# PJLab-ADG/nr3d_lib

Hardware: AMD Instinct MI355X
Metric: Mpoints/s LoTD fwd+bwd (16-lvl hash) + Mrays/s march+composite, 1 & 8 GPU (higher is better)
Workload: dtype f32; 1 GPU; configs[1]: 16-level Hash LoTD (gen_ngp_cfg: T=2^19, F=2, 6 Dense + 10 Hash), 2^20 points/GPU, fwd(+dy/dx) + dL/dx + dL/dparam, fp32; points_per_gpu=1048576, n_params=12131648, parallelism=single GPU

## Files before the change

include/nr3d_hip.h:

```cpp
#ifndef NR3D_HIP_H
#define NR3D_HIP_H
#include <stdint.h>

#ifdef __cplusplus
extern "C" {
#endif

enum { NR3D_F32 = 0, NR3D_F16 = 1, NR3D_F64 = 2, NR3D_I32 = 3, NR3D_I64 = 4, NR3D_U8 = 5, NR3D_I16 = 6, NR3D_I8 = 7 };

#define NR3D_ABI_VERSION 16

const char *nr3d_last_error(void);
int nr3d_abi_version(void);

enum {
	NR3D_PROF_LOTD_FWD = 0,
	NR3D_PROF_LOTD_FWD_LDS = 1,
	NR3D_PROF_LOTD_CONTRACT_DX = 2,
	NR3D_PROF_LOTD_BIN = 3,
	NR3D_PROF_LOTD_ACCUM = 4,
	NR3D_PROF_MARCH = 5,
	NR3D_PROF_COMPOSITE_FWD = 6,
	NR3D_PROF_COMPOSITE_BWD = 7,
	NR3D_PROF_LOTD_DIRECT = 8,
	NR3D_PROF_COUNT = 9
};
void nr3d_prof_enable(uint32_t mask);
int nr3d_prof_read(int id, double *total_ms, uint32_t *n_intervals, int reset);

enum {
	NR3D_OPT_LOTD_PAIR = 0,
	NR3D_OPT_PAIR_QUAD = 1,
	NR3D_OPT_PAIR_SECOND = 2,
	NR3D_OPT_PAIR_DIRECT = 3,
	NR3D_OPT_PAIR_FIXED = 4,
	NR3D_OPT_FWD_PAIRLANE = 5,
	NR3D_OPT_FWD_SPLIT = 6,
	NR3D_OPT_FWD_LDS_STAGE = 7,
	NR3D_OPT_HVP_LEVELS = 8,
	NR3D_OPT_HVP_PAIRLANE = 9,
	NR3D_OPT_HVP_SPLIT = 10,
	NR3D_OPT_VM_SPLIT = 11,
	NR3D_OPT_CP_DIRECT = 12,
	NR3D_OPT_MARCH_GROUP = 13,
	NR3D_OPT_PACK_SCAN = 14,
	NR3D_OPT_SORT_WAVE = 15,
	NR3D_OPT_VM_DIRECT = 16,
	NR3D_OPT_DIRECT_FIXED = 17,
	NR3D_OPT_VM_SORTED = 18,
	NR3D_OPT_MLP_X3 = 19,
	NR3D_OPT_PAIR_FOLD = 20,
	NR3D_OPT_COUNT = 21
};
int nr3d_set_option(int id, int64_t value);
int64_t nr3d_get_option(int id);

#define NR3D_LOTD_MAX_LEVELS 32
#define NR3D_LOTD_MAX_DIMS 4
#define NR3D_LOTD_MAX_PSEUDO 256

enum {
	NR3D_LOD_Dense = 0, NR3D_LOD_VectorMatrix = 1, NR3D_LOD_VecZMatXoY = 2, NR3D_LOD_CP = 3,
	NR3D_LOD_CPfast = 4, NR3D_LOD_NPlaneMul = 5, NR3D_LOD_NPlaneSum = 6, NR3D_LOD_Hash = 7
};

typedef struct nr3d_lotd_level {
	uint32_t res[NR3D_LOTD_MAX_DIMS];
	uint32_t n_feats;
	uint32_t type;
	uint32_t size;
	uint32_t offset;
} nr3d_lotd_level_t;

typedef struct nr3d_lotd_meta {
	nr3d_lotd_level_t levels[NR3D_LOTD_MAX_LEVELS];
	uint16_t map_levels[NR3D_LOTD_MAX_PSEUDO];
	uint16_t map_cnt[NR3D_LOTD_MAX_PSEUDO];
	uint32_t n_levels;
	uint32_t n_pseudo_levels;
	uint32_t n_feat_per_pseudo_lvl;
	uint32_t n_dims_to_encode;
	uint32_t n_encoded_dims;
	uint32_t n_params;
	uint32_t interpolation_type;
	uint32_t c_hash_only;
	uint16_t map_col[NR3D_LOTD_MAX_PSEUDO];
} nr3d_lotd_meta_t;

int nr3d_lotd_meta_create(int32_t n_input_dim, uint32_t n_levels, const int32_t *res_multidim,
                          const int32_t *n_feats, const int32_t *types, uint32_t hashmap_size,
                          int use_smooth_step, nr3d_lotd_meta_t *out);

int nr3d_lotd_meta_regroup(const nr3d_lotd_meta_t *meta, uint32_t width, uint32_t max_width, nr3d_lotd_meta_t *out);


int nr3d_lotd_fwd(const nr3d_lotd_meta_t *meta, const void *meta_dev, uint32_t n_points,
                  int x_dtype, int param_dtype, const void *x, const void *params,
                  const int64_t *batch_inds, const int64_t *batch_offsets, uint32_t batch_data_size,
                  int32_t max_level, void *y, int64_t y_sn, int64_t y_se,
                  void *dy_dx, int64_t dydx_sn, int64_t dydx_se, void *stream);

int nr3d_lotd_bwd_dx(const nr3d_lotd_meta_t *meta, uint32_t n_points, int x_dtype, int param_dtype,
                     const void *dL_dy, int64_t dldy_sn, int64_t dldy_se,
                     const void *dy_dx, int64_t dydx_sn, int64_t dydx_se, void *dL_dx,
                     void *dL_dy_T ,
                     int32_t max_level, void *fold ,
                     void *stream);

uint64_t nr3d_lotd_dparam_workspace_bytes(const nr3d_lotd_meta_t *meta, uint32_t n_points, uint32_t n_batches);
void nr3d_lotd_set_dparam_chunk_log2(int log2_points);
int nr3d_lotd_bwd_dparam(const nr3d_lotd_meta_t *meta, const void *meta_dev, uint32_t n_points,
                         int x_dtype, int param_dtype, const void *dL_dy, int64_t dldy_sn, int64_t dldy_se,
                         const void *x, const void *params, const int64_t *batch_inds,
                         const int64_t *batch_offsets, uint32_t batch_data_size, uint32_t n_batches, int32_t max_level,
                         void *dL_dparam, void *workspace, uint64_t workspace_bytes, void *stream);
int nr3d_lotd_bwd_dparam_levels(const nr3d_lotd_meta_t *meta, const void *meta_dev, uint32_t n_points,
                                int x_dtype, int param_dtype, const void *dL_dy, int64_t dldy_sn, int64_t dldy_se,
                                const void *x, const void *params, const int64_t *batch_inds,
                                const int64_t *batch_offsets, uint32_t batch_data_size, uint32_t n_batches,
                                int32_t min_level, int32_t max_level, void *dL_dparam, void *workspace,
                                uint64_t workspace_bytes, void *stream);

int nr3d_lotd_dLdy_feature_major(uint32_t n_points, uint32_t n_encoded_dims, int grad_dtype, const void *dL_dy,
                                 int64_t g_sn, int64_t g_se, float *out, void *stream);

int nr3d_lotd_half_params_ok(const nr3d_lotd_meta_t *meta, int batched);
int nr3d_lotd_pair_path_ok(const nr3d_lotd_meta_t *meta);
int nr3d_lotd_pair_direct_levels(const nr3d_lotd_meta_t *meta, uint32_t n_points);
uint64_t nr3d_lotd_fwd_lds_levels(const nr3d_lotd_meta_t *meta, uint32_t n_points);
int nr3d_lotd_bwd_dparam_typed(const nr3d_lotd_meta_t *meta, const void *meta_dev, uint32_t n_points, int grad_dtype,
                               const void *dL_dy, int64_t g_sn, int64_t g_se, const void *x, int32_t max_level,
                               int out_dtype, int assign, void *dL_dparam, void *workspace, uint64_t workspace_bytes,
                               void *fold, void *stream);
uint64_t nr3d_lotd_pair_fold_bytes(const nr3d_lotd_meta_t *meta, uint32_t n_points, int32_t max_level);

int nr3d_lotd_bwd_bwd_ddLdy(const nr3d_lotd_meta_t *meta, uint32_t n_points, int x_dtype, int param_dtype,
                            const void *dL_ddLdx, const void *dy_dx, int64_t dydx_sn, int64_t dydx_se,
                            void *dL_ddLdy, int64_t out_sn, int64_t out_se, void *stream);
int nr3d_lotd_bwd_bwd_dparam(const nr3d_lotd_meta_t *meta, const void *meta_dev, uint32_t n_points,
                             int x_dtype, int param_dtype, const void *dL_ddLdx,
                             const void *dL_dy, int64_t dldy_sn, int64_t dldy_se, const void *x,
                             const void *params, const int64_t *batch_inds, const int64_t *batch_offsets,
                             uint32_t batch_data_size, uint32_t n_batches, int32_t max_level, void *dL_dparam,
                             void *workspace, uint64_t workspace_bytes, void *stream);
uint64_t nr3d_lotd_bwd_bwd_dx_workspace_bytes(const nr3d_lotd_meta_t *meta, uint32_t n_points);
int nr3d_lotd_bwd_bwd_dx(const nr3d_lotd_meta_t *meta, const void *meta_dev, uint32_t n_points,
                         int x_dtype, int param_dtype, const void *dL_ddLdx,
                         const void *dL_dy, int64_t dldy_sn, int64_t dldy_se, const void *x,
                         const void *params, const int64_t *batch_inds, const int64_t *batch_offsets,
                         uint32_t batch_data_size, int32_t max_level, void *dL_dx, void *workspace,
                         uint64_t workspace_bytes, void *stream);

int nr3d_lotd_grid_index(const nr3d_lotd_meta_t *meta, const void *meta_dev, uint32_t n_points, int x_dtype,
                         const void *x, const int64_t *batch_inds, const int64_t *batch_offsets,
                         uint32_t batch_data_size, int32_t max_level, int64_t *grid_inds, void *stream);

typedef struct nr3d_forest_meta {
	const uint8_t *octree;
	const int32_t *exsum;
	const int16_t *block_ks;
	float world_block_size[3];
	float world_origin[3];
	int32_t resolution[3];
	uint32_t n_trees;
	uint32_t level;
	uint32_t level_poffset;
	int32_t continuity_enabled;
} nr3d_forest_meta_t;

int nr3d_forest_identify(const nr3d_forest_meta_t *forest, uint64_t n, const int16_t *ks, int32_t *block_inds,
                         void *stream);

int nr3d_lotd_forest_fwd(const nr3d_lotd_meta_t *meta, const void *meta_dev, const nr3d_forest_meta_t *forest,
                         uint32_t n_points, const float *x, const void *params, int param_dtype ,
                         const int64_t *block_inds,
                         const int64_t *block_offsets, uint32_t batch_data_size, int32_t max_level, float *y,
                         int64_t y_sn, int64_t y_se, float *dy_dx, int64_t d_sn, int64_t d_se, void *stream);

uint64_t nr3d_lotd_forest_dparam_workspace_bytes(const nr3d_lotd_meta_t *meta, uint32_t n_points, uint32_t n_trees);
int nr3d_lotd_forest_bwd_dparam(const nr3d_lotd_meta_t *meta, const void *meta_dev, const nr3d_forest_meta_t *forest,
                                uint32_t n_points, const float *dL_ddLdx, const float *dL_dy, const float *x,
                                const void *params, int param_dtype, const int64_t *block_inds, const int64_t *block_offsets,
                                uint32_t batch_data_size, int32_t max_level, float *dL_dparam, void *workspace,
                                uint64_t workspace_bytes, void *stream);

int nr3d_lotd_forest_bwd_bwd_dx(const nr3d_lotd_meta_t *meta, const void *meta_dev, const nr3d_forest_meta_t *forest,
// ... 288 lines not shown
```

nr3d_lib_amd/_abi.py:

```python
ABI_VERSION = 16
SIGNATURES = {
    'nr3d_abi_version': ('int', []),
    'nr3d_alpha_to_vw_backward': ('int', ['uint32_t', 'uint64_t', 'ptr', 'ptr', 'ptr', 'ptr', 'float', 'float', 'ptr', 'ptr']),
    'nr3d_alpha_to_vw_forward': ('int', ['uint32_t', 'uint64_t', 'ptr', 'ptr', 'float', 'float', 'ptr', 'ptr', 'ptr', 'ptr']),
    'nr3d_arange_num_steps': ('int', ['uint32_t', 'int', 'ptr', 'ptr', 'ptr', 'double', 'ptr', 'ptr']),
    'nr3d_forest_identify': ('int', ['ptr', 'uint64_t', 'ptr', 'ptr', 'ptr']),
    'nr3d_forest_ray_marching_count': ('int', ['ptr', 'uint32_t', 'ptr', 'ptr', 'ptr', 'ptr', 'ptr', 'ptr', 'ptr', 'ptr', 'ptr', 'ptr', 'float', 'float', 'float', 'uint32_t', 'ptr', 'ptr', 'ptr', 'ptr']),
    'nr3d_forest_ray_marching_emit': ('int', ['ptr', 'uint32_t', 'ptr', 'ptr', 'ptr', 'ptr', 'ptr', 'ptr', 'ptr', 'ptr', 'ptr', 'ptr', 'float', 'float', 'float', 'ptr', 'ptr', 'ptr', 'ptr', 'ptr', 'ptr', 'ptr']),
    'nr3d_freq_encode_bwd': ('int', ['uint64_t', 'uint32_t', 'uint32_t', 'uint32_t', 'ptr', 'ptr', 'int64_t', 'ptr', 'ptr']),
    'nr3d_freq_encode_bwd_bwd': ('int', ['uint64_t', 'uint32_t', 'uint32_t', 'uint32_t', 'ptr', 'ptr', 'ptr', 'int64_t', 'ptr', 'ptr', 'ptr']),
    'nr3d_freq_encode_fwd': ('int', ['uint64_t', 'uint32_t', 'uint32_t', 'uint32_t', 'ptr', 'ptr', 'int64_t', 'ptr']),
    'nr3d_get_option': ('int64_t', ['int']),
    'nr3d_interleave_linstep': ('int', ['uint32_t', 'int', 'ptr', 'ptr', 'ptr', 'double', 'double', 'ptr', 'ptr', 'ptr']),
    'nr3d_last_error': ('str', []),
    'nr3d_lotd_bwd_bwd_ddLdy': ('int', ['ptr', 'uint32_t', 'int', 'int', 'ptr', 'ptr', 'int64_t', 'int64_t', 'ptr', 'int64_t', 'int64_t', 'ptr']),
    'nr3d_lotd_bwd_bwd_dparam': ('int', ['ptr', 'ptr', 'uint32_t', 'int', 'int', 'ptr', 'ptr', 'int64_t', 'int64_t', 'ptr', 'ptr', 'ptr', 'ptr', 'uint32_t', 'uint32_t', 'int32_t', 'ptr', 'ptr', 'uint64_t', 'ptr']),
    'nr3d_lotd_bwd_bwd_dx': ('int', ['ptr', 'ptr', 'uint32_t', 'int', 'int', 'ptr', 'ptr', 'int64_t', 'int64_t', 'ptr', 'ptr', 'ptr', 'ptr', 'uint32_t', 'int32_t', 'ptr', 'ptr', 'uint64_t', 'ptr']),
    'nr3d_lotd_bwd_bwd_dx_workspace_bytes': ('uint64_t', ['ptr', 'uint32_t']),
    'nr3d_lotd_bwd_dparam': ('int', ['ptr', 'ptr', 'uint32_t', 'int', 'int', 'ptr', 'int64_t', 'int64_t', 'ptr', 'ptr', 'ptr', 'ptr', 'uint32_t', 'uint32_t', 'int32_t', 'ptr', 'ptr', 'uint64_t', 'ptr']),
    'nr3d_lotd_bwd_dparam_levels': ('int', ['ptr', 'ptr', 'uint32_t', 'int', 'int', 'ptr', 'int64_t', 'int64_t', 'ptr', 'ptr', 'ptr', 'ptr', 'uint32_t', 'uint32_t', 'int32_t', 'int32_t', 'ptr', 'ptr', 'uint64_t', 'ptr']),
    'nr3d_lotd_bwd_dparam_typed': ('int', ['ptr', 'ptr', 'uint32_t', 'int', 'ptr', 'int64_t', 'int64_t', 'ptr', 'int32_t', 'int', 'int', 'ptr', 'ptr', 'uint64_t', 'ptr', 'ptr']),
    'nr3d_lotd_bwd_dx': ('int', ['ptr', 'uint32_t', 'int', 'int', 'ptr', 'int64_t', 'int64_t', 'ptr', 'int64_t', 'int64_t', 'ptr', 'ptr', 'int32_t', 'ptr', 'ptr']),
    'nr3d_lotd_dLdy_feature_major': ('int', ['uint32_t', 'uint32_t', 'int', 'ptr', 'int64_t', 'int64_t', 'ptr', 'ptr']),
    'nr3d_lotd_dparam_workspace_bytes': ('uint64_t', ['ptr', 'uint32_t', 'uint32_t']),
    'nr3d_lotd_forest_bwd_bwd_dx': ('int', ['ptr', 'ptr', 'ptr', 'uint32_t', 'ptr', 'ptr', 'ptr', 'ptr', 'int', 'ptr', 'ptr', 'uint32_t', 'int32_t', 'ptr', 'ptr']),
    'nr3d_lotd_forest_bwd_dparam': ('int', ['ptr', 'ptr', 'ptr', 'uint32_t', 'ptr', 'ptr', 'ptr', 'ptr', 'int', 'ptr', 'ptr', 'uint32_t', 'int32_t', 'ptr', 'ptr', 'uint64_t', 'ptr']),
    'nr3d_lotd_forest_dparam_workspace_bytes': ('uint64_t', ['ptr', 'uint32_t', 'uint32_t']),
    'nr3d_lotd_forest_fwd': ('int', ['ptr', 'ptr', 'ptr', 'uint32_t', 'ptr', 'ptr', 'int', 'ptr', 'ptr', 'uint32_t', 'int32_t', 'ptr', 'int64_t', 'int64_t', 'ptr', 'int64_t', 'int64_t', 'ptr']),
    'nr3d_lotd_fwd': ('int', ['ptr', 'ptr', 'uint32_t', 'int', 'int', 'ptr', 'ptr', 'ptr', 'ptr', 'uint32_t', 'int32_t', 'ptr', 'int64_t', 'int64_t', 'ptr', 'int64_t', 'int64_t', 'ptr']),
    'nr3d_lotd_fwd_lds_levels': ('uint64_t', ['ptr', 'uint32_t']),
    'nr3d_lotd_grid_index': ('int', ['ptr', 'ptr', 'uint32_t', 'int', 'ptr', 'ptr', 'ptr', 'uint32_t', 'int32_t', 'ptr', 'ptr']),
    'nr3d_lotd_half_params_ok': ('int', ['ptr', 'int']),
    'nr3d_lotd_meta_create': ('int', ['int32_t', 'uint32_t', 'ptr', 'ptr', 'ptr', 'uint32_t', 'int', 'ptr']),
    'nr3d_lotd_meta_regroup': ('int', ['ptr', 'uint32_t', 'uint32_t', 'ptr']),
    'nr3d_lotd_pair_direct_levels': ('int', ['ptr', 'uint32_t']),
    'nr3d_lotd_pair_fold_bytes': ('uint64_t', ['ptr', 'uint32_t', 'int32_t']),
    'nr3d_lotd_pair_path_ok': ('int', ['ptr']),
    'nr3d_lotd_set_dparam_chunk_log2': ('void', ['int']),
    'nr3d_march_composite_bwd': ('int', ['uint32_t', 'ptr', 'ptr', 'ptr', 'ptr', 'ptr', 'float', 'float', 'int', 'ptr', 'ptr', 'ptr', 'ptr', 'ptr', 'ptr', 'ptr', 'ptr', 'ptr', 'ptr', 'uint64_t', 'ptr', 'ptr']),
    'nr3d_march_composite_fwd': ('int', ['uint32_t', 'ptr', 'ptr', 'ptr', 'ptr', 'ptr', 'ptr', 'ptr', 'int', 'float', 'float', 'float', 'uint32_t', 'ptr', 'ptr', 'ptr', 'ptr', 'ptr', 'ptr', 'uint64_t', 'uint64_t', 'ptr', 'ptr', 'ptr', 'ptr', 'ptr', 'ptr', 'ptr', 'ptr', 'uint64_t', 'ptr', 'float', 'float', 'int', 'ptr', 'ptr', 'ptr', 'ptr', 'ptr', 'ptr']),
    'nr3d_march_finish_samples': ('int', ['uint64_t', 'ptr', 'ptr', 'ptr', 'ptr', 'ptr', 'ptr', 'ptr', 'ptr', 'ptr']),
    'nr3d_mark_pack_boundaries': ('int', ['uint64_t', 'int', 'ptr', 'ptr', 'ptr']),
    'nr3d_merge_pack_union': ('int', ['uint32_t', 'ptr', 'ptr', 'uint32_t', 'ptr', 'ptr', 'ptr', 'ptr', 'ptr', 'ptr', 'ptr', 'ptr', 'ptr', 'ptr', 'ptr', 'ptr']),
    'nr3d_mlp_backward': ('int', ['ptr', 'uint64_t', 'ptr', 'int64_t', 'int64_t', 'ptr', 'int64_t', 'ptr', 'ptr', 'int64_t', 'int64_t', 'ptr', 'ptr', 'ptr']),
    'nr3d_mlp_backward_backward': ('int', ['ptr', 'uint64_t', 'ptr', 'int64_t', 'int64_t', 'ptr', 'int64_t', 'ptr', 'int64_t', 'int64_t', 'ptr', 'ptr', 'int64_t', 'ptr', 'ptr']),
    'nr3d_mlp_backward_backward_ok': ('int', ['ptr']),
    'nr3d_mlp_backward_packed_floats': ('uint64_t', ['ptr']),
    'nr3d_mlp_forward': ('int', ['ptr', 'uint64_t', 'ptr', 'int64_t', 'int64_t', 'ptr', 'ptr', 'int64_t', 'ptr']),
    'nr3d_mlp_half_backward': ('int', ['ptr', 'uint64_t', 'ptr', 'int64_t', 'int64_t', 'ptr', 'int64_t', 'ptr', 'ptr', 'int64_t', 'int64_t', 'ptr', 'ptr', 'ptr']),
    'nr3d_mlp_half_backward_packed_bytes': ('uint64_t', ['ptr']),
    'nr3d_mlp_half_forward': ('int', ['ptr', 'uint64_t', 'ptr', 'int64_t', 'int64_t', 'ptr', 'ptr', 'int64_t', 'ptr']),
    'nr3d_mlp_half_pack': ('int', ['ptr', 'ptr', 'ptr', 'ptr', 'int', 'ptr']),
    'nr3d_mlp_half_packed_bytes': ('uint64_t', ['ptr']),
    'nr3d_mlp_pack': ('int', ['ptr', 'ptr', 'ptr', 'ptr', 'int', 'ptr']),
    'nr3d_mlp_packed_floats': ('uint64_t', ['ptr']),
    'nr3d_occ_apply_max': ('int', ['uint64_t', 'float', 'ptr', 'ptr', 'ptr']),
    'nr3d_occ_scatter_max': ('int', ['uint64_t', 'ptr', 'ptr', 'ptr', 'uint64_t', 'ptr', 'ptr', 'uint32_t', 'ptr', 'ptr']),
    'nr3d_octree_mark_consecutive_segments': ('int', ['uint32_t', 'ptr', 'ptr', 'ptr', 'ptr', 'ptr', 'ptr']),
    'nr3d_order_gather_inputs': ('int', ['uint32_t', 'ptr', 'ptr', 'ptr', 'ptr', 'ptr', 'ptr', 'ptr', 'ptr']),
    'nr3d_order_move_rows': ('int', ['uint32_t', 'ptr', 'int', 'ptr', 'uint32_t', 'ptr', 'ptr', 'uint32_t', 'ptr', 'ptr']),
    'nr3d_pack_composite_bwd': ('int', ['uint32_t', 'ptr', 'ptr', 'ptr', 'ptr', 'ptr', 'ptr', 'float', 'float', 'int', 'ptr', 'ptr', 'ptr', 'ptr', 'ptr', 'ptr', 'ptr', 'ptr', 'ptr', 'ptr']),
    'nr3d_pack_composite_fwd': ('int', ['uint32_t', 'ptr', 'ptr', 'ptr', 'ptr', 'ptr', 'float', 'float', 'int', 'ptr', 'ptr', 'ptr', 'ptr', 'ptr']),
    'nr3d_pack_infos_from_n': ('int', ['uint32_t', 'ptr', 'ptr', 'ptr', 'ptr', 'ptr']),
    'nr3d_packed_binary': ('int', ['uint32_t', 'uint64_t', 'uint32_t', 'uint32_t', 'int', 'ptr', 'ptr', 'ptr', 'int', 'int', 'ptr', 'ptr']),
    'nr3d_packed_diff': ('int', ['uint32_t', 'uint64_t', 'uint32_t', 'int', 'ptr', 'ptr', 'ptr', 'ptr', 'int', 'int', 'ptr', 'ptr']),
    'nr3d_packed_invert_cdf': ('int', ['uint32_t', 'ptr', 'ptr', 'ptr', 'ptr', 'uint32_t', 'ptr', 'ptr', 'ptr']),
    'nr3d_packed_scan': ('int', ['uint32_t', 'uint64_t', 'uint32_t', 'int', 'ptr', 'ptr', 'int', 'int', 'int', 'int', 'ptr', 'ptr']),
    'nr3d_packed_searchsorted': ('int', ['uint32_t', 'int', 'ptr', 'ptr', 'ptr', 'uint32_t', 'ptr', 'ptr', 'ptr']),
    'nr3d_packed_sort': ('int', ['uint32_t', 'uint64_t', 'int', 'ptr', 'ptr', 'ptr', 'ptr']),
    'nr3d_packed_sum': ('int', ['uint32_t', 'uint64_t', 'uint32_t', 'int', 'ptr', 'ptr', 'ptr', 'ptr']),
    'nr3d_permuto_bwd': ('int', ['ptr', 'uint32_t', 'int', 'ptr', 'int64_t', 'int64_t', 'ptr', 'ptr', 'ptr', 'ptr', 'ptr', 'ptr', 'uint32_t', 'int32_t', 'uint32_t', 'ptr', 'ptr', 'ptr']),
    'nr3d_permuto_bwd_bwd_input': ('int', ['ptr', 'uint32_t', 'int', 'ptr', 'ptr', 'int64_t', 'int64_t', 'ptr', 'ptr', 'ptr', 'ptr', 'ptr', 'ptr', 'uint32_t', 'int32_t', 'ptr', 'int64_t', 'int64_t', 'ptr', 'ptr']),
    'nr3d_permuto_fwd': ('int', ['ptr', 'uint32_t', 'int', 'ptr', 'ptr', 'ptr', 'ptr', 'ptr', 'ptr', 'uint32_t', 'int32_t', 'ptr', 'int64_t', 'int64_t', 'ptr']),
    'nr3d_permuto_meta_create': ('int', ['int32_t', 'int32_t', 'uint32_t', 'ptr', 'ptr', 'ptr', 'ptr']),
    'nr3d_permuto_supported_n_input_dims': ('int', ['ptr']),
    'nr3d_prof_enable': ('void', ['uint32_t']),
    'nr3d_prof_read': ('int', ['int', 'ptr', 'ptr', 'int']),
    'nr3d_prune_compact_packs': ('int', ['uint32_t', 'ptr', 'ptr', 'ptr', 'ptr', 'ptr', 'ptr', 'ptr', 'ptr']),
    'nr3d_prune_compact_samples': ('int', ['uint32_t', 'ptr', 'ptr', 'ptr', 'ptr', 'ptr', 'ptr', 'ptr', 'ptr', 'ptr', 'ptr', 'ptr', 'ptr', 'ptr']),
    'nr3d_ray_marching_cache_bytes': ('uint64_t', ['uint32_t', 'uint32_t']),
    'nr3d_ray_marching_count': ('int', ['uint32_t', 'ptr', 'ptr', 'ptr', 'ptr', 'ptr', 'ptr', 'ptr', 'int', 'float', 'float', 'float', 'uint32_t', 'int', 'ptr', 'uint32_t', 'ptr', 'ptr', 'ptr', 'ptr', 'uint64_t', 'ptr']),
    'nr3d_ray_marching_count_finished': ('int', ['uint32_t', 'ptr', 'ptr', 'ptr', 'ptr', 'ptr', 'ptr', 'ptr', 'int', 'float', 'float', 'float', 'uint32_t', 'int', 'ptr', 'uint32_t', 'ptr', 'ptr', 'ptr', 'ptr', 'ptr', 'ptr', 'uint64_t', 'ptr']),
    'nr3d_ray_marching_emit': ('int', ['uint32_t', 'ptr', 'ptr', 'ptr', 'ptr', 'ptr', 'ptr', 'ptr', 'int', 'float', 'float', 'float', 'int', 'ptr', 'uint32_t', 'ptr', 'ptr', 'ptr', 'ptr', 'ptr', 'ptr', 'ptr', 'uint32_t', 'ptr']),
    'nr3d_ray_marching_emit_finished': ('int', ['uint32_t', 'ptr', 'ptr', 'int', 'ptr', 'uint32_t', 'ptr', 'ptr', 'uint32_t', 'ptr', 'ptr', 'ptr', 'ptr', 'ptr', 'ptr', 'ptr', 'ptr', 'ptr']),
    'nr3d_sample_step_count': ('int', ['uint32_t', 'ptr', 'ptr', 'uint32_t', 'float', 'float', 'float', 'ptr', 'ptr']),
    'nr3d_sample_step_emit': ('int', ['uint32_t', 'ptr', 'ptr', 'float', 'float', 'float', 'ptr', 'ptr', 'ptr', 'ptr']),
    'nr3d_sample_step_segments': ('int', ['uint32_t', 'ptr', 'ptr', 'ptr', 'ptr', 'ptr', 'uint32_t', 'float', 'float', 'float', 'int', 'ptr', 'ptr', 'ptr', 'ptr', 'ptr', 'ptr', 'ptr']),
    'nr3d_scan_tmp_bytes': ('uint64_t', ['uint64_t']),
    'nr3d_set_option': ('int', ['int', 'int64_t']),
    'nr3d_sh_encode_bwd': ('int', ['uint64_t', 'uint32_t', 'uint32_t', 'int', 'ptr', 'int64_t', 'ptr', 'ptr', 'ptr', 'int', 'ptr']),
# ... 24 lines not shown
```

nr3d_lib_amd/_hip.py:

```python
import ctypes as C
import os
import subprocess
import threading

import torch

from nr3d_lib_amd import _abi

_PKG = os.path.dirname(os.path.abspath(__file__))
LIB_PATH = os.path.join(_PKG, "libnr3d_hip.so")
ABI_VERSION = _abi.ABI_VERSION
CSRC = os.path.join(_PKG, "csrc")

F32, F16, F64, I32, I64, U8, I16, I8 = range(8)
DTYPE_CODE = {
    torch.float32: F32, torch.float16: F16, torch.float64: F64, torch.int32: I32, torch.int64: I64,
    torch.uint8: U8, torch.bool: U8, torch.int16: I16, torch.int8: I8,
}

_lib = None
_lock = threading.Lock()


def build(verbose=False, jobs=None):
# ... 53 lines not shown
    if missing:
        raise RuntimeError(f"nr3d_lib_amd: {LIB_PATH} does not export {missing} (stale build? `make -C nr3d_lib_amd/csrc`)")


POISON = os.environ.get("NR3D_POISON_EMPTY", "0") == "1"


def _poison(t):
    if t.numel() == 0:
        return t
    if t.dtype.is_floating_point:
        t.fill_(float("nan"))
    elif t.dtype == torch.bool:
        t.fill_(True)
    else:
        t.fill_(-0x54545455 if t.dtype in (torch.int32, torch.int64) else 0x2B)
    return t


def empty(*args, **kwargs):
    t = torch.empty(*args, **kwargs)
    return _poison(t) if POISON else t


def empty_like(x, **kwargs):
    t = torch.empty_like(x, **kwargs)
    return _poison(t) if POISON else t


def check(rc):
    if rc != 0:
        raise RuntimeError(lib().nr3d_last_error().decode())


PROF_IDS = dict(lotd_fwd=0, lotd_fwd_lds=1, lotd_contract_dx=2, lotd_bin=3, lotd_accum=4, march=5, composite_fwd=6,
                composite_bwd=7, lotd_direct=8)


def prof_enable(*names):
    mask = 0
    for n in names:
        mask |= 1 << PROF_IDS[n]
    lib().nr3d_prof_enable(mask)


def prof_read(name, reset=True):
    ms, n = C.c_double(0.0), C.c_uint32(0)
    check(lib().nr3d_prof_read(PROF_IDS[name], C.byref(ms), C.byref(n), 1 if reset else 0))
    return float(ms.value), int(n.value)


OPTION_IDS = dict(lotd_pair=0, pair_quad=1, pair_second=2, pair_direct=3, pair_fixed=4, fwd_pairlane=5, fwd_split=6,
                  fwd_lds_stage=7, hvp_levels=8, hvp_pairlane=9, hvp_split=10, vm_split=11, cp_direct=12, march_group=13,
                  pack_scan=14, sort_wave=15, vm_direct=16, direct_fixed=17, vm_sorted=18, mlp_x3=19, pair_fold=20)


def set_option(name, value):
    l = lib()
    check(l.nr3d_set_option(OPTION_IDS[name], -1 if value is None else int(value)))


def get_option(name):
    l = lib()
    return int(l.nr3d_get_option(OPTION_IDS[name]))


class options:

    def __init__(self, **kw):
        self.kw, self.old = kw, {}

    def __enter__(self):
        for k, v in self.kw.items():
            self.old[k] = get_option(k)
            set_option(k, v)
        return self

    def __exit__(self, *a):
        for k, v in self.old.items():
            set_option(k, v)
        return False


def ptr(t):
    if t is None:
        return None
    return t.data_ptr()


_raw_stream = getattr(torch._C, "_cuda_getCurrentRawStream", None)


def stream_of(t):
    if _raw_stream is not None:
        return _raw_stream(t.device.index if t.device.index is not None else torch.cuda.current_device())
    return torch.cuda.current_stream(t.device).cuda_stream


def sort_pairs_u32(keys, values=None, bits=32, n_dev=None):
    pair = isinstance(keys, (list, tuple))
    ks = list(keys) if pair else [keys]
    vs = list(values) if isinstance(values, (list, tuple)) else [values] * len(ks)
    assert len(ks) in (1, 2) and all(k.is_cuda and k.dtype == torch.int32 and k.is_contiguous() and k.shape == ks[0].shape for k in ks)
    assert all(v is None or (v.is_cuda and v.dtype == torch.int32 and v.is_contiguous() and v.shape == ks[0].shape) for v in vs)
    n, dev = ks[0].numel(), ks[0].device
    l = lib()
    tmp = torch.empty(int(l.nr3d_sort_pairs_u32_tmp_bytes(n, len(ks))) or 1, dtype=torch.uint8, device=dev)
# ... 155 lines not shown
```

nr3d_lib_amd/bindings/_forest.py:

```python
import ctypes as C

import torch

from .. import _hip as H

__all__ = ['ForestMeta', 'forest_identify']


class _CForest(C.Structure):
    _fields_ = [("octree", C.c_void_p), ("exsum", C.c_void_p), ("block_ks", C.c_void_p),
                ("world_block_size", C.c_float * 3), ("world_origin", C.c_float * 3), ("resolution", C.c_int32 * 3),
                ("n_trees", C.c_uint32), ("level", C.c_uint32), ("level_poffset", C.c_uint32),
                ("continuity_enabled", C.c_int32)]


class ForestMeta:

    def __init__(self):
        self.octree = None
        self.exsum = None
        self.block_ks = None
        self.world_block_size = [1.0, 1.0, 1.0]
        self.world_origin = [0.0, 0.0, 0.0]
        self.resolution = [1, 1, 1]
# ... 68 lines not shown
            need_input_grad=None):
    from . import _lotd
    m, fo, N, bds = _check("fwd", metas, input, params, batch_inds, batch_offsets, batch_data_size)
    max_level = m.n_levels if max_level is None else int(max_level)
    need_input_grad = bool(input.requires_grad) if need_input_grad is None else bool(need_input_grad)
    E, dev = m.n_encoded_dims, input.device
    if max_level <= -1:
        return (torch.zeros((N, E), dtype=params.dtype, device=dev), torch.zeros((N, E * 3), dtype=input.dtype, device=dev))
    x32, (p32, pcode) = _lotd._f32c(input.detach()), _lotd._ptab(params)
    with H.on_device(dev):
        y = H.empty((E, N), dtype=torch.float32, device=dev).t()
        dy_dx, dsn, dse = None, 0, 0
        if need_input_grad:
            if m.c_permute_dydx:
                dy_dx = H.empty((E, N, 3), dtype=torch.float32, device=dev).permute(1, 0, 2)
                dsn, dse = dy_dx.stride(0), dy_dx.stride(1)
            else:
                dy_dx, dsn, dse = H.empty((N, E * 3), dtype=torch.float32, device=dev), E * 3, 3
        c = fo._c()
        H.check(H.lib().nr3d_lotd_forest_fwd(
            C.byref(m._cmeta()), H.ptr(m._dev(dev)), C.byref(c), N, H.ptr(x32), H.ptr(p32), pcode, H.ptr(batch_inds),
            H.ptr(batch_offsets), bds, max_level, H.ptr(y), y.stride(0), y.stride(1), H.ptr(dy_dx), dsn, dse, H.stream_of(input)))
    return _lotd._cast(y, params.dtype), _lotd._cast(dy_dx, input.dtype)


def lod_bwd(metas, dL_dy, input, params, dy_dx=None, batch_inds=None, batch_offsets=None, batch_data_size=None,
            max_level=None, need_input_grad=None, need_param_grad=None):
    from . import _lotd
    m, fo, N, bds = _check("bwd", metas, input, params, batch_inds, batch_offsets, batch_data_size)
    E, dev = m.n_encoded_dims, input.device
    H.require_gpu(dL_dy, dy_dx)
    if tuple(dL_dy.shape) != (N, E):
        raise RuntimeError(f"bwd: Expected dL_dy of size [{N}, {E}], got {list(dL_dy.shape)}")
    if dL_dy.dtype != params.dtype:
        raise RuntimeError("bwd: Expected dL_dy and grid to have the same dtype")
    max_level = m.n_levels if max_level is None else int(max_level)
    need_input_grad = bool(input.requires_grad) if need_input_grad is None else bool(need_input_grad)
    need_param_grad = bool(params.requires_grad) if need_param_grad is None else bool(need_param_grad)
    dL_dx = dL_dparam = None
    with H.on_device(dev):
        if need_input_grad:
            if dy_dx is None:
                raise RuntimeError("LoTDEncoding::bwd: need `dy_dx` to comput `dL_dx`.")
            dL_dx = torch.zeros((N, 3), dtype=torch.float32, device=dev)
        if need_param_grad:
            dL_dparam = torch.zeros((params.shape[0],), dtype=torch.float32, device=dev)
        if max_level <= -1 or N == 0 or not (need_input_grad or need_param_grad):
            return _lotd._cast(dL_dx, input.dtype), _lotd._cast(dL_dparam, params.dtype)
        g32 = _lotd._f32c(dL_dy.detach()).contiguous()
        st = H.stream_of(input)
        if need_input_grad:
            j, jsn, jse = _lotd._jac_view(dy_dx.detach(), N, E, 3)
            H.check(H.lib().nr3d_lotd_bwd_dx(
                C.byref(m._cmeta()), N, H.F32, H.F32, H.ptr(g32), E, 1, H.ptr(j), jsn, jse, H.ptr(dL_dx), None, max_level, None,
                st))
        if need_param_grad:
            x32, (p32, pcode) = _lotd._f32c(input.detach()), _lotd._ptab(params)
            c = fo._c()
            ws, wsb = _workspace(m, fo, N, dev)
            H.check(H.lib().nr3d_lotd_forest_bwd_dparam(
                C.byref(m._cmeta()), H.ptr(m._dev(dev)), C.byref(c), N, None, H.ptr(g32), H.ptr(x32), H.ptr(p32), pcode,
                H.ptr(batch_inds), H.ptr(batch_offsets), bds, max_level, H.ptr(dL_dparam), H.ptr(ws), wsb, st))
    return _lotd._cast(dL_dx, input.dtype), _lotd._cast(dL_dparam, params.dtype)


def lod_bwd_bwd_input(metas, dL_ddLdx, dL_dy, input, params, dy_dx=None, batch_inds=None, batch_offsets=None,
                      batch_data_size=None, max_level=None, need_dLdinput_ddLdoutput=None, need_dLdinput_dparams=None,
                      need_dLdinput_dinput=None):
    from . import _lotd
    m, fo, N, bds = _check("bwd_bwd_input", metas, input, params, batch_inds, batch_offsets, batch_data_size)
    E, dev = m.n_encoded_dims, input.device
    H.require_gpu(dL_ddLdx, dL_dy, dy_dx)
    if input.dtype != torch.float32:
        raise RuntimeError("LoTDEncoding: Input type combination not supported. Supported types are: "
                           "<input,param> -> (half, half), (float, half), (float, float)")
    if tuple(dL_ddLdx.shape) != (N, 3) or not dL_ddLdx.is_contiguous() or dL_ddLdx.dtype != input.dtype:
        raise RuntimeError(f"bwd_bwd_input: Expected contiguous dL_ddLdx of size [{N}, 3] and the input's dtype")
    if tuple(dL_dy.shape) != (N, E) or dL_dy.dtype != params.dtype:
        raise RuntimeError(f"bwd_bwd_input: Expected dL_dy of size [{N}, {E}] and the params' dtype")
    max_level = m.n_levels if max_level is None else int(max_level)
    need_dLdy = bool(dL_dy.requires_grad) if need_dLdinput_ddLdoutput is None else bool(need_dLdinput_ddLdoutput)
    need_dx = bool(input.requires_grad) if need_dLdinput_dinput is None else bool(need_dLdinput_dinput)
    need_dp = bool(params.requires_grad) if need_dLdinput_dparams is None else bool(need_dLdinput_dparams)
    dL_ddLdy = dL_dparams = dL_dx = None
    with H.on_device(dev):
        if need_dLdy:
            if dy_dx is None:
                raise RuntimeError("LoTDEncoding::bwd_bwd_input: need `dy_dx` to compute `dL_d(dLdy)`.")
            dL_ddLdy = torch.zeros((N, E), dtype=torch.float32, device=dev)
        if need_dx:
            dL_dx = torch.zeros((N, 3), dtype=torch.float32, device=dev)
        if need_dp:
            dL_dparams = torch.zeros((params.shape[0],), dtype=torch.float32, device=dev)
        if max_level <= -1 or N == 0 or not (need_dLdy or need_dx or need_dp):
            return _lotd._cast(dL_ddLdy, dL_dy.dtype), _lotd._cast(dL_dparams, params.dtype), _lotd._cast(dL_dx, input.dtype)
        st = H.stream_of(input)
        v32, g32 = _lotd._f32c(dL_ddLdx.detach()), _lotd._f32c(dL_dy.detach()).contiguous()
        x32, (p32, pcode) = _lotd._f32c(input.detach()), _lotd._ptab(params)
        cm, md, c = C.byref(m._cmeta()), H.ptr(m._dev(dev)), fo._c()
        if need_dLdy:
            j, jsn, jse = _lotd._jac_view(dy_dx.detach(), N, E, 3)
            H.check(H.lib().nr3d_lotd_bwd_bwd_ddLdy(
                cm, N, H.F32, H.F32, H.ptr(v32), H.ptr(j), jsn, jse, H.ptr(dL_ddLdy), E, 1, st))
        if need_dx:
            H.check(H.lib().nr3d_lotd_forest_bwd_bwd_dx(
                cm, md, C.byref(c), N, H.ptr(v32), H.ptr(g32), H.ptr(x32), H.ptr(p32), pcode, H.ptr(batch_inds),
                H.ptr(batch_offsets), bds, max_level, H.ptr(dL_dx), st))
# ... 11 lines not shown
```

nr3d_lib_amd/bindings/_lotd.py:

```python
import ctypes as C
import enum

import torch

from .. import _hip as H

MAX_LEVELS, MAX_DIMS, MAX_PSEUDO = 32, 4, 256


class LoDType(enum.IntEnum):
    Dense = 0
    VectorMatrix = 1
    VecZMatXoY = 2
    CP = 3
    CPfast = 4
    NPlaneMul = 5
    NPlaneSum = 6
    Hash = 7


class InterpolationType(enum.IntEnum):
    Linear = 0
    Smoothstep = 1

# ... 297 lines not shown
    if dy_dx is not None and input.dtype != torch.float32:
        dy_dx = dy_dx.to(input.dtype)
    return y, dy_dx


def lod_bwd(lod_meta, dL_dy, input, params, dy_dx=None, batch_inds=None, batch_offsets=None, batch_data_size=None,
            max_level=None, need_input_grad=None, need_param_grad=None, level_buckets=None, on_bucket=None):
    if isinstance(lod_meta, tuple):
        from . import _forest
        return _forest.lod_bwd(lod_meta, dL_dy, input, params, dy_dx, batch_inds, batch_offsets, batch_data_size, max_level,
                               need_input_grad, need_param_grad)
    m = lod_meta
    N, bds = _check_common("bwd", m, input, params, batch_inds, batch_offsets, batch_data_size)
    E, D = m.n_encoded_dims, m.n_dims_to_encode
    H.require_gpu(dL_dy, dy_dx)
    if dL_dy.dim() != 2 or tuple(dL_dy.shape) != (N, E):
        raise RuntimeError(f"bwd: Expected dL_dy of size [{N}, {E}], got {list(dL_dy.shape)}")
    if dL_dy.dtype != params.dtype:
        raise RuntimeError("bwd: Expected dL_dy and grid to have the same dtype")
    if dy_dx is not None and dy_dx.dtype != input.dtype:
        raise RuntimeError("bwd: Expected x and dy_dx to have the same dtype")
    max_level = m.n_levels if max_level is None else int(max_level)
    need_input_grad = bool(input.requires_grad) if need_input_grad is None else bool(need_input_grad)
    need_param_grad = bool(params.requires_grad) if need_param_grad is None else bool(need_param_grad)
    dev = input.device
    dL_dx = dL_dparam = None
    with H.on_device(dev):
        if need_input_grad and dy_dx is None:
            raise RuntimeError("LoTDEncoding::bwd: need `dy_dx` to comput `dL_dx`.")
        batched = batch_inds is not None or batch_offsets is not None or bds != 0
        nothing = max_level <= -1 or not (need_input_grad or need_param_grad) or N == 0
        native = (_native_half(m, params, batched) and level_buckets is None and USE_BINNED_DPARAM and input.dtype == torch.float32
                  and dL_dy.is_contiguous() and E % 4 == 0 and dL_dy.data_ptr() % 8 == 0 and not nothing
                  and params.shape[0] == m.n_params)
        typed = (not nothing and not batched and level_buckets is None and USE_BINNED_DPARAM
                 and (native or params.dtype == torch.float32) and params.shape[0] == m.n_params
                 and bool(H.lib().nr3d_lotd_pair_path_ok(C.byref(m._cmeta()))))
        if need_input_grad:
            dL_dx = (torch.zeros if nothing else H.empty)((N, D), dtype=torch.float32, device=dev)
        if need_param_grad:
            dL_dparam = (H.empty if typed else torch.zeros)((params.shape[0],), dtype=torch.float16 if native else torch.float32,
                                                                device=dev)
        if nothing:
            if need_param_grad and level_buckets is not None and on_bucket is not None:
                for k, (lo, hi) in enumerate(level_buckets):
                    on_bucket(k, dL_dparam[m.level_offsets[int(lo)]:m.level_offsets[min(int(hi), m.n_levels - 1) + 1]])
            return (_cast(dL_dx, input.dtype), _cast(dL_dparam, params.dtype))
        g32 = dL_dy.detach() if native else _f32c(dL_dy.detach())
        gcode = H.F16 if native else H.F32
        gsn, gse = _strides2(g32)
        st = H.stream_of(input)
        tag = ("dx" if need_input_grad else "") + ("dp" if need_param_grad else "")
        with _Prof(m, f"LoTD{D}-bwd-{tag}", N):
            gT = fold = None
            if need_input_grad and N > 0:
                j, jsn, jse = _jac_view(dy_dx.detach(), N, E, D)
                if (need_param_grad and not batched and USE_BINNED_DPARAM and gse == 1 and gsn == E
                        and g32.data_ptr() % 16 == 0):
                    gT = H.empty((E, N), dtype=torch.float32, device=dev)
                    if typed:
                        nfold = H.lib().nr3d_lotd_pair_fold_bytes(C.byref(m._cmeta()), N, max_level)
                        if nfold:
                            fold = H.empty(((nfold + 3) // 4,), dtype=torch.int32, device=dev)
                H.check(H.lib().nr3d_lotd_bwd_dx(
                    C.byref(m._cmeta()), N, H.F32, gcode, H.ptr(g32), gsn, gse, H.ptr(j), jsn, jse, H.ptr(dL_dx), H.ptr(gT),
                    max_level, H.ptr(fold), st))
            if need_param_grad and N > 0 and typed:
                ws, wsb = _dparam_workspace(m, N, dev, 1)
                if gT is not None:
                    g32, gsn, gse, gcode = gT, 1, N, H.F32
                H.check(H.lib().nr3d_lotd_bwd_dparam_typed(
                    C.byref(m._cmeta()), H.ptr(m._dev(dev)), N, gcode, H.ptr(g32), gsn, gse, H.ptr(_f32c(input.detach())),
                    max_level, H.F16 if native else H.F32, 1, H.ptr(dL_dparam), H.ptr(ws), wsb, H.ptr(fold), st))
            elif need_param_grad and N > 0:
                x32, (p32, pcode) = _f32c(input.detach()), _ptab(params)
                nbat = _n_batches(m, p32, batch_offsets, batched)
                ws, wsb = _dparam_workspace(m, N, dev, nbat)
                if gT is not None:
                    g32, gsn, gse = gT, 1, N
                if level_buckets is None:
                    H.check(H.lib().nr3d_lotd_bwd_dparam(
                        C.byref(m._cmeta()), H.ptr(m._dev(dev)), N, H.F32, pcode, H.ptr(g32), gsn, gse, H.ptr(x32), H.ptr(p32),
                        H.ptr(batch_inds), H.ptr(batch_offsets), bds, nbat, max_level, H.ptr(dL_dparam), H.ptr(ws), wsb, st))
                else:
                    if batched:
                        raise RuntimeError("bwd: level_buckets need non-batched params")
                    if params.dtype != torch.float32:
                        raise RuntimeError("bwd: level_buckets need float params (the slices handed out are the result)")
                    seen = set()
                    for k, (lo, hi) in enumerate(level_buckets):
                        lo, hi = int(lo), min(int(hi), m.n_levels - 1)
                        if lo < 0 or lo > hi or seen & set(range(lo, hi + 1)):
                            raise RuntimeError(f"bwd: bad or overlapping level bucket {(lo, hi)}")
                        seen |= set(range(lo, hi + 1))
                        H.check(H.lib().nr3d_lotd_bwd_dparam_levels(
                            C.byref(m._cmeta()), H.ptr(m._dev(dev)), N, H.F32, H.F32, H.ptr(g32), gsn, gse, H.ptr(x32), H.ptr(p32),
                            None, None, 0, nbat, lo, min(hi, max_level), H.ptr(dL_dparam), H.ptr(ws), wsb, st))
                        if on_bucket is not None:
                            on_bucket(k, dL_dparam[m.level_offsets[lo]:m.level_offsets[hi + 1]])
    return _cast(dL_dx, input.dtype), _cast(dL_dparam, params.dtype)


def _cast(t, dtype):
    if t is None or t.dtype == dtype:
        return t
    return t.to(dtype)


def lod_bwd_bwd_input(lod_meta, dL_ddLdx, dL_dy, input, params, dy_dx=None, batch_inds=None, batch_offsets=None,
                      batch_data_size=None, max_level=None, need_dLdinput_ddLdoutput=None,
                      need_dLdinput_dparams=None, need_dLdinput_dinput=None):
    if isinstance(lod_meta, tuple):
        from . import _forest
        return _forest.lod_bwd_bwd_input(lod_meta, dL_ddLdx, dL_dy, input, params, dy_dx, batch_inds, batch_offsets,
                                         batch_data_size, max_level, need_dLdinput_ddLdoutput, need_dLdinput_dparams,
                                         need_dLdinput_dinput)
    m = lod_meta
    N, bds = _check_common("bwd_bwd_input", m, input, params, batch_inds, batch_offsets, batch_data_size)
    E, D = m.n_encoded_dims, m.n_dims_to_encode
    H.require_gpu(dL_ddLdx, dL_dy, dy_dx)
    if input.dtype != torch.float32:
        raise RuntimeError("LoTDEncoding: Input type combination not supported. Supported types are: "
                           "<input,param> -> (half, half), (float, half), (float, float)")
    if tuple(dL_ddLdx.shape) != (N, D) or not dL_ddLdx.is_contiguous() or dL_ddLdx.dtype != input.dtype:
        raise RuntimeError(f"bwd_bwd_input: Expected contiguous dL_ddLdx of size [{N}, {D}] and the input's dtype")
    if tuple(dL_dy.shape) != (N, E) or dL_dy.dtype != params.dtype:
# ... 78 lines not shown
```

nr3d_lib_amd/csrc/host_api.hip:

```cpp
#include "common.h"
#include <string.h>
#include <limits>
#include <chrono>
#include <mutex>
#include <vector>

namespace nr3d {

static thread_local char g_err[512] = {0};

char *err_buf() { return g_err; }

int fail(const char *fmt, ...) {
	va_list ap;
	va_start(ap, fmt);
	vsnprintf(g_err, sizeof(g_err), fmt, ap);
	va_end(ap);
	return 1;
}

namespace prof {
uint32_t g_mask = 0;
struct Pair { hipEvent_t a, b; };
static std::mutex g_mu;
static std::vector<Pair> g_done[NR3D_PROF_COUNT];
static std::vector<Pair> g_free;
static Pair g_open[NR3D_PROF_COUNT];
static bool g_is_open[NR3D_PROF_COUNT] = {};

void begin(int id, hipStream_t st) {
	std::lock_guard<std::mutex> lk(g_mu);
	if (id < 0 || id >= NR3D_PROF_COUNT || g_is_open[id]) return;
	Pair p;
	if (!g_free.empty()) { p = g_free.back(); g_free.pop_back(); }
	else if (hipEventCreate(&p.a) != hipSuccess || hipEventCreate(&p.b) != hipSuccess) return;
	if (hipEventRecord(p.a, st) != hipSuccess) return;
	g_open[id] = p; g_is_open[id] = true;
}
void end(int id, hipStream_t st) {
	std::lock_guard<std::mutex> lk(g_mu);
	if (id < 0 || id >= NR3D_PROF_COUNT || !g_is_open[id]) return;
	g_is_open[id] = false;
	if (hipEventRecord(g_open[id].b, st) == hipSuccess) g_done[id].push_back(g_open[id]);
}
}

namespace opt {
static const int64_t kDefault[NR3D_OPT_COUNT] = {
	 1,  1,  1,  1,  1,  1,
	 1,  1,  1,  1,  1,  1,
	 1,  0,  1,  1,  1,  1,
	 1,  1,  1,
};
std::atomic<int64_t> g_val[NR3D_OPT_COUNT];
static const bool g_val_init = [] {
	for (int i = 0; i < NR3D_OPT_COUNT; ++i) g_val[i].store(kDefault[i], std::memory_order_relaxed);
	return true;
}();
}

}

using namespace nr3d;

extern "C" void nr3d_prof_enable(uint32_t mask) { prof::g_mask = mask; }

extern "C" int nr3d_prof_read(int id, double *total_ms, uint32_t *n_intervals, int reset) {
	NR3D_CHECK(id >= 0 && id < NR3D_PROF_COUNT && total_ms && n_intervals, "prof_read: bad argument");
	std::lock_guard<std::mutex> lk(prof::g_mu);
	double sum = 0.0;
	for (const prof::Pair &p : prof::g_done[id]) {
		NR3D_HIP_CHECK(hipEventSynchronize(p.b));
		float ms = 0.0f;
		NR3D_HIP_CHECK(hipEventElapsedTime(&ms, p.a, p.b));
		sum += ms;
	}
	*total_ms = sum;
	*n_intervals = (uint32_t)prof::g_done[id].size();
	if (reset) {
		for (const prof::Pair &p : prof::g_done[id]) prof::g_free.push_back(p);
		prof::g_done[id].clear();
	}
	return 0;
}

extern "C" int nr3d_set_option(int id, int64_t value) {
	NR3D_CHECK(id >= 0 && id < NR3D_OPT_COUNT, "nr3d_set_option: unknown option %d", id);
	opt::g_val[id].store(value < 0 ? opt::kDefault[id] : value, std::memory_order_relaxed);
	return 0;
}
extern "C" int64_t nr3d_get_option(int id) { return (id >= 0 && id < NR3D_OPT_COUNT) ? opt::get(id) : -1; }

extern "C" int nr3d_wait_host_words(const int64_t *words, int n, int64_t sentinel, uint32_t timeout_us) {
	if (!words || n <= 0) return 0;
	const auto t0 = std::chrono::steady_clock::now();
	for (uint32_t spin = 0;; ++spin) {
		bool all = true;
		for (int i = 0; i < n; ++i)
			if (__atomic_load_n(&words[i], __ATOMIC_ACQUIRE) == sentinel) { all = false; break; }
		if (all) return 0;
		__builtin_ia32_pause();
		if ((spin & 63u) == 63u &&
		    std::chrono::duration_cast<std::chrono::microseconds>(std::chrono::steady_clock::now() - t0).count() > (int64_t)timeout_us)
			return 1;
	}
// ... 129 lines not shown
```

nr3d_lib_amd/csrc/lotd.hip:

```cpp
#include "lotd_device.h"
#include <stdlib.h>
#include <vector>
#include <type_traits>
#include <algorithm>

namespace nr3d {
namespace lotd {

template <typename YT> __device__ __forceinline__ void store_nt(YT *p, float v);

template <int D, int G, bool DYDX, bool DH, int ONLY = -1, typename PT = float>
__global__ __launch_bounds__(kBlock) void k_fwd(Sched s, const nr3d_lotd_meta_t *__restrict__ md, uint32_t N,
                                                int32_t max_level, uint32_t smooth, const float *__restrict__ x,
                                                const PT *__restrict__ params, Batch ba, uint32_t vec_ok,
                                                PT *__restrict__ y, int64_t y_sn, int64_t y_se,
                                                float *__restrict__ dydx, int64_t d_sn, int64_t d_se) {
	uint32_t q, chunk;
	if (!decode_block(s, blockIdx.x, q, chunk)) return;
	const uint32_t i = chunk * kBlock + threadIdx.x;
	if (i >= N) return;
	const uint32_t level = meta_level_of(md, q);
	const uint32_t foff0 = meta_cnt_of(md, q) * G;
	const uint32_t out0 = meta_col_of(md, q);

// ... 955 lines not shown
			float *dst = reinterpret_cast<float *>(reinterpret_cast<char *>(partial) + ((size_t)q * N + g0) * 12u + pl * 12u);
			__builtin_nontemporal_store(ox[u], &dst[0]);
			__builtin_nontemporal_store(oy[u], &dst[1]);
			__builtin_nontemporal_store(oz[u], &dst[2]);
		}
	}
}

template <int D>
__global__ __launch_bounds__(kBlock) void k_sum_levels(uint32_t N, uint32_t n_pseudo, const float *__restrict__ partial,
                                                       float *__restrict__ dL_dx) {
	const uint32_t i = blockIdx.x * kBlock + threadIdx.x;
	if (i >= N) return;
	float acc[D];
#pragma unroll
	for (int d = 0; d < D; ++d) acc[d] = 0.0f;
	for (uint32_t q = 0; q < n_pseudo; ++q) {
		const float *src = partial + ((size_t)q * N + i) * D;
#pragma unroll
		for (int d = 0; d < D; ++d) acc[d] += __builtin_nontemporal_load(src + d);
	}
#pragma unroll
	for (int d = 0; d < D; ++d) dL_dx[(size_t)i * D + d] = acc[d];
}


template <int D>
__global__ __launch_bounds__(kBlock) void k_contract_dx(uint32_t N, uint32_t E, const float *__restrict__ dL_dy,
                                                        int64_t g_sn, int64_t g_se, const float *__restrict__ dydx,
                                                        int64_t d_sn, int64_t d_se, float *__restrict__ dL_dx) {
	const uint32_t i = blockIdx.x * kBlock + threadIdx.x;
	if (i >= N) return;
	float acc[D];
#pragma unroll
	for (int d = 0; d < D; ++d) acc[d] = 0.0f;
	const float *gy = dL_dy + (int64_t)i * g_sn;
	const float *jj = dydx + (int64_t)i * d_sn;
#pragma unroll 4
	for (uint32_t e = 0; e < E; ++e) {
		const float g = gy[(int64_t)e * g_se];
		const float *j = jj + (int64_t)e * d_se;
#pragma unroll
		for (int d = 0; d < D; ++d) acc[d] = __fmaf_rn(g, j[d], acc[d]);
	}
#pragma unroll
	for (int d = 0; d < D; ++d) dL_dx[(size_t)i * D + d] = acc[d];
}

template <int D, typename GT>
__global__ __launch_bounds__(kBlock) void k_contract_dx_rowmajor(uint32_t N, uint32_t E, const GT *__restrict__ dL_dy,
                                                                 const float *__restrict__ dydx, int64_t d_sn,
                                                                 int64_t d_se, float *__restrict__ dL_dx,
                                                                 float *__restrict__ dL_dy_T, uint32_t *__restrict__ fold,
                                                                 uint32_t gcols, uint32_t n_zero, uint32_t slot_off) {
	constexpr int TE = 32;
	__shared__ float tile[TE][kBlock + 1];
	__shared__ uint32_t gred[kBlock / 64];
	const uint32_t i0 = blockIdx.x * kBlock, i = i0 + threadIdx.x;
	const uint32_t n_here = min((uint32_t)kBlock, N - i0);
	uint32_t gbits = 0;
	auto gm = [&](uint32_t e, float v) { if (e < gcols) gbits = max(gbits, __float_as_uint(v) & 0x7FFFFFFFu); };
	if (fold && blockIdx.x == 0)
		for (uint32_t k = threadIdx.x; k < n_zero; k += kBlock) fold[k] = 0u;
	float acc[D];
#pragma unroll
	for (int d = 0; d < D; ++d) acc[d] = 0.0f;
	for (uint32_t e0 = 0; e0 < E; e0 += TE) {
		const uint32_t te = min((uint32_t)TE, E - e0);
		if (te == TE && (E & 3u) == 0u) {
#pragma unroll
			for (uint32_t v = threadIdx.x; v < kBlock * TE / 4; v += kBlock) {
				const uint32_t p = v >> 3, e4 = (v & 7u) * 4u;
				if (p < n_here) {
					float4 t;
					if constexpr (sizeof(GT) == 4) {
						t = *reinterpret_cast<const float4 *>(dL_dy + (size_t)(i0 + p) * E + e0 + e4);
					} else {
						const __half2 *h = reinterpret_cast<const __half2 *>(dL_dy + (size_t)(i0 + p) * E + e0 + e4);
						const float2 a = __half22float2(h[0]), b = __half22float2(h[1]);
						t = make_float4(a.x, a.y, b.x, b.y);
					}
					tile[e4][p] = t.x; tile[e4 + 1][p] = t.y; tile[e4 + 2][p] = t.z; tile[e4 + 3][p] = t.w;
					if (fold) { gm(e0 + e4, t.x); gm(e0 + e4 + 1, t.y); gm(e0 + e4 + 2, t.z); gm(e0 + e4 + 3, t.w); }
				}
			}
		} else {
			for (uint32_t v = threadIdx.x; v < kBlock * te; v += kBlock) {
				const uint32_t p = v / te, e = v - p * te;
				if (p < n_here) {
					tile[e][p] = to_f32<GT>(dL_dy[(size_t)(i0 + p) * E + e0 + e]);
					if (fold) gm(e0 + e, tile[e][p]);
				}
			}
		}
		__syncthreads();
		if (dL_dy_T && i < N) {
#pragma unroll 8
			for (uint32_t e = 0; e < te; ++e) __builtin_nontemporal_store(tile[e][threadIdx.x], &dL_dy_T[(size_t)(e0 + e) * N + i]);
		}
		if (i < N) {
			const float *jj = dydx + (int64_t)i * d_sn + (int64_t)e0 * d_se;
#pragma unroll 8
			for (uint32_t e = 0; e < te; ++e) {
				const float g = tile[e][threadIdx.x];
				const float *j = jj + (int64_t)e * d_se;
#pragma unroll
				for (int d = 0; d < D; ++d) acc[d] = __fmaf_rn(g, __builtin_nontemporal_load(j + d), acc[d]);
			}
		}
		__syncthreads();
	}
	if (i < N) {
#pragma unroll
		for (int d = 0; d < D; ++d) dL_dx[(size_t)i * D + d] = acc[d];
	}
	if (fold) {
#pragma unroll
		for (int off = 32; off >= 1; off >>= 1) gbits = max(gbits, (uint32_t)__shfl_xor((int)gbits, off, 64));
		if ((threadIdx.x & 63u) == 0) gred[threadIdx.x >> 6] = gbits;
		__syncthreads();
		if (threadIdx.x == 0) {
#pragma unroll
			for (int k = 1; k < kBlock / 64; ++k) gbits = max(gbits, gred[k]);
			fold[slot_off + blockIdx.x] = gbits;
		}
	}
}

template <int D>
__global__ __launch_bounds__(kBlock) void k_contract_ddLdy(uint32_t N, uint32_t E, const float *__restrict__ v,
                                                           const float *__restrict__ dydx, int64_t d_sn, int64_t d_se,
                                                           float *__restrict__ out, int64_t o_sn, int64_t o_se) {
	const uint32_t i = blockIdx.x * kBlock + threadIdx.x;
	const uint32_t e = blockIdx.y;
	if (i >= N) return;
	const float *j = dydx + (int64_t)i * d_sn + (int64_t)e * d_se;
	float r = 0.0f;
#pragma unroll
	for (int d = 0; d < D; ++d) r = __fmaf_rn(v[(size_t)i * D + d], j[d], r);
	out[(int64_t)i * o_sn + (int64_t)e * o_se] = r;
}

template <int D, int G>
__global__ __launch_bounds__(kBlock) void k_grid_index(Sched s, const nr3d_lotd_meta_t *__restrict__ md, uint32_t N,
                                                       uint32_t E, int32_t max_level, const float *__restrict__ x,
                                                       Batch ba, int64_t *__restrict__ out) {
	uint32_t q, chunk;
	if (!decode_block(s, blockIdx.x, q, chunk)) return;
	const uint32_t i = chunk * kBlock + threadIdx.x;
	if (i >= N) return;
	const uint32_t level = meta_level_of(md, q);
// ... 294 lines not shown
                       hipStream_t st) {
	uint32_t n_blocks;
	const Batch ba{batch_inds, batch_offsets, batch_data_size, meta->n_params};
	const uint32_t G = meta->n_feat_per_pseudo_lvl;
	const uint32_t elt = p_half ? 2u : 4u;
	const uint32_t vec_ok = (((uintptr_t)params % ((G >= 4 ? 4u : 2u) * elt)) == 0 && batch_offsets == nullptr) ? 1u : 0u;
	const bool dh = meta->c_hash_only != 0;
	prof::Scope ps(NR3D_PROF_LOTD_FWD, st);
	uint64_t grp[4] = {0, 0, 0, 0};
	const bool split = !dh && meta->n_pseudo_levels <= 64u && opt::on(NR3D_OPT_FWD_SPLIT);
	const uint64_t all = meta->n_pseudo_levels >= 64u ? ~0ull : ((1ull << meta->n_pseudo_levels) - 1ull);
	if (split) {
		for (uint32_t q = 0; q < meta->n_pseudo_levels; ++q) {
			const uint32_t t = meta->levels[meta->map_levels[q]].type;
			int k = 0;
			if (t == NR3D_LOD_Dense || t == NR3D_LOD_Hash) k = 1;
			else if (meta->n_dims_to_encode == 3 && t == NR3D_LOD_CP) k = 2;
			else if (meta->n_dims_to_encode == 3 && t == NR3D_LOD_VectorMatrix) k = 3;
			grp[k] |= 1ull << q;
		}
	} else {
		grp[dh ? 1 : 0] = all;
	}
	for (int k = 0; k < 4; ++k) {
		if (!grp[k]) continue;
		const uint64_t skip = (split || meta->n_pseudo_levels <= 64u) ? (all & ~grp[k]) : 0ull;
		const Sched s = make_sched(N, meta, n_blocks, skip);
		if (n_blocks == 0) continue;
		DISPATCH_DG(meta->n_dims_to_encode, G, {
			auto launch = [&](auto kern_f32, auto kern_f16) {
				if (p_half)
					hipLaunchKernelGGL(kern_f16, dim3(n_blocks), dim3(kBlock), 0, st, s, md, N, max_level,
					                   meta->interpolation_type, (const float *)x, (const __half *)params, ba, vec_ok,
					                   (__half *)y, y_sn, y_se, (float *)dy_dx, d_sn, d_se);
				else
					hipLaunchKernelGGL(kern_f32, dim3(n_blocks), dim3(kBlock), 0, st, s, md, N, max_level,
					                   meta->interpolation_type, (const float *)x, (const float *)params, ba, vec_ok,
					                   (float *)y, y_sn, y_se, (float *)dy_dx, d_sn, d_se);
			};
			if (k == 1) { if (dy_dx) NR3D_FWD2(D, true, true, -1); else NR3D_FWD2(D, false, true, -1); }
			else if (k == 0) { if (dy_dx) NR3D_FWD2(D, true, false, -1); else NR3D_FWD2(D, false, false, -1); }
			else if constexpr (D == 3) {
				if (k == 2) { if (dy_dx) NR3D_FWD2(3, true, false, NR3D_LOD_CP); else NR3D_FWD2(3, false, false, NR3D_LOD_CP); }
				else { if (dy_dx) NR3D_FWD2(3, true, false, NR3D_LOD_VectorMatrix); else NR3D_FWD2(3, false, false, NR3D_LOD_VectorMatrix); }
			}
		});
	}
	NR3D_LAUNCH_CHECK();
	return 0;
}

extern "C" int nr3d_lotd_bwd_dx(const nr3d_lotd_meta_t *meta, uint32_t N, int x_dtype, int param_dtype, const void *dL_dy,
                                int64_t g_sn, int64_t g_se, const void *dy_dx, int64_t d_sn, int64_t d_se, void *dL_dx,
                                void *dL_dy_T, int32_t max_level, void *fold_buf, void *stream) {
	NR3D_CHECK(meta != nullptr, "LoTD: meta is NULL");
	NR3D_CHECK(x_dtype == NR3D_F32 && (param_dtype == NR3D_F32 || param_dtype == NR3D_F16), "LoTD::bwd_dx: f32 x, f32 / f16 dL_dy");
	if (N == 0) return 0;
	NR3D_CHECK(dL_dy && dy_dx && dL_dx, "LoTDEncoding::bwd: need `dy_dx` to comput `dL_dx`.");
	const uint32_t E = meta->n_encoded_dims;
	const bool g_half = param_dtype == NR3D_F16;
	const bool row_major = (g_se == 1 && g_sn == (int64_t)E && ((uintptr_t)dL_dy % (g_half ? 8 : 16)) == 0);
	NR3D_CHECK(dL_dy_T == nullptr || row_major, "LoTD::bwd_dx: dL_dy_T needs a contiguous, 16-byte aligned [N, E] dL_dy");
	NR3D_CHECK(!g_half || (row_major && (E & 3u) == 0u), "LoTD::bwd_dx: half dL_dy must be a contiguous [N, E] tensor, E % 4 == 0");
	uint32_t gcols = 0, n_zero = 0, slot_off = 0;
	uint32_t *fold = (fold_buf && pair_fold_layout(meta, N, max_level, gcols, n_zero, slot_off) != 0) ? (uint32_t *)fold_buf : nullptr;
	NR3D_CHECK(!fold || row_major, "LoTD::bwd_dx: the hand-over buffer needs a contiguous, 16-byte aligned [N, E] dL_dy");
	prof::Scope ps(NR3D_PROF_LOTD_CONTRACT_DX, (hipStream_t)stream);
	DISPATCH_D(meta->n_dims_to_encode, {
		if (row_major && g_half)
			hipLaunchKernelGGL((k_contract_dx_rowmajor<D, __half>), dim3(div_up(N, kBlock)), dim3(kBlock), 0, (hipStream_t)stream, N, E,
			                   (const __half *)dL_dy, (const float *)dy_dx, d_sn, d_se, (float *)dL_dx, (float *)dL_dy_T, fold, gcols,
			                   n_zero, slot_off);
		else if (row_major)
			hipLaunchKernelGGL((k_contract_dx_rowmajor<D, float>), dim3(div_up(N, kBlock)), dim3(kBlock), 0, (hipStream_t)stream, N, E,
			                   (const float *)dL_dy, (const float *)dy_dx, d_sn, d_se, (float *)dL_dx, (float *)dL_dy_T, fold, gcols,
			                   n_zero, slot_off);
		else
			hipLaunchKernelGGL(k_contract_dx<D>, dim3(div_up(N, kBlock)), dim3(kBlock), 0, (hipStream_t)stream, N, E,
			                   (const float *)dL_dy, g_sn, g_se, (const float *)dy_dx, d_sn, d_se, (float *)dL_dx);
	});
	NR3D_LAUNCH_CHECK();
	return 0;
}

extern "C" uint64_t nr3d_lotd_pair_fold_bytes(const nr3d_lotd_meta_t *meta, uint32_t N, int32_t max_level) {
	uint32_t gcols, n_zero, slot_off;
	return meta ? pair_fold_layout(meta, N, max_level, gcols, n_zero, slot_off) : 0;
}

static int launch_bwd_dparam(const DparamPass &p) {
	const nr3d_lotd_meta_t *meta = p.meta;
	if (p.N == 0 || p.max_level <= -1 || p.min_level > p.max_level) return 0;
	NR3D_CHECK(p.dL_dy && p.x && p.params && p.dparam, "LoTD::bwd: NULL tensor pointer");
	const bool batched = p.batch.inds || p.batch.offsets || p.batch.data_size;
	if (p.workspace && (!batched || p.n_batches > 0)) {
		bool handled = false;
		DparamPass q = p;
		if (!batched) q.n_batches = 1u;
		NR3D_TRY(dparam_binned(q, handled));
		if (handled) return 0;
	}
	uint32_t n_blocks;
	const Sched s = make_sched(p.N, meta, n_blocks);
	const bool dh = meta->c_hash_only != 0;
	DISPATCH_DG(meta->n_dims_to_encode, meta->n_feat_per_pseudo_lvl, {
		auto launch = [&](auto kern, auto *tab) {
			hipLaunchKernelGGL(kern, dim3(n_blocks), dim3(kBlock), 0, p.st, s, p.meta_dev, p.N, p.min_level, p.max_level,
			                   meta->interpolation_type, p.dL_ddLdx, p.dL_dy, p.g_sn, p.g_se, p.x, tab, p.batch, p.dparam);
		};
		const float *pf = (const float *)p.params;
		if (dh || !p.p_half)
			with_bool(p.second, [&](auto S) { if (dh) launch(k_bwd_dparam<D, G, S(), true>, pf); else launch(k_bwd_dparam<D, G, S(), false>, pf); });
		else with_bool(p.second, [&](auto S) { launch(k_bwd_dparam<D, G, S(), false, __half>, (const __half *)p.params); });
	});
	NR3D_LAUNCH_CHECK();
	return 0;
}

extern "C" int nr3d_lotd_bwd_dparam(const nr3d_lotd_meta_t *meta, const void *meta_dev, uint32_t N, int x_dtype,
                                    int param_dtype, const void *dL_dy, int64_t g_sn, int64_t g_se, const void *x,
                                    const void *params, const int64_t *batch_inds, const int64_t *batch_offsets,
                                    uint32_t batch_data_size, uint32_t n_batches, int32_t max_level, void *dL_dparam,
                                    void *workspace, uint64_t workspace_bytes, void *stream) {
	if (int rc = check_common(meta, meta_dev, x_dtype, param_dtype, true)) return rc;
	DparamPass p = plain_pass(meta, meta_dev, N, dL_dy, g_sn, g_se, x, dL_dparam);
	p.params = params; p.p_half = param_dtype == NR3D_F16;
	p.batch = Batch{batch_inds, batch_offsets, batch_data_size, meta->n_params}; p.n_batches = n_batches;
	p.min_level = 0; p.max_level = max_level;
	p.workspace = workspace; p.workspace_bytes = workspace_bytes; p.st = (hipStream_t)stream;
	return launch_bwd_dparam(p);
}

extern "C" int nr3d_lotd_pair_path_ok(const nr3d_lotd_meta_t *meta) { return (meta && pair_applies(meta)) ? 1 : 0; }
extern "C" uint64_t nr3d_lotd_fwd_lds_levels(const nr3d_lotd_meta_t *meta, uint32_t n_points) {
	if (!meta || !pairlane_enabled() || !pairlane_meta_ok(meta)) return 0;
	return fwd_lds_levels(meta, n_points, 0x7fffffff);
}

extern "C" int nr3d_lotd_pair_direct_levels(const nr3d_lotd_meta_t *meta, uint32_t n_points) {
	return (meta && pair_applies(meta)) ? (int)pair_direct_levels(meta, n_points) : 0;
}

extern "C" int nr3d_lotd_bwd_dparam_typed(const nr3d_lotd_meta_t *meta, const void *meta_dev, uint32_t N, int grad_dtype,
                                          const void *dL_dy, int64_t g_sn, int64_t g_se, const void *x, int32_t max_level,
                                          int out_dtype, int assign, void *dL_dparam, void *workspace, uint64_t workspace_bytes,
                                          void *fold, void *stream) {
	if (int rc = check_common(meta, meta_dev, NR3D_F32, NR3D_F32)) return rc;
	NR3D_CHECK((grad_dtype == NR3D_F32 || grad_dtype == NR3D_F16) && (out_dtype == NR3D_F32 || out_dtype == NR3D_F16),
	           "LoTD::bwd_dparam_typed: f32 / f16 only");
	if (N == 0 || max_level <= -1) {
		if (assign && dL_dparam)
			NR3D_HIP_CHECK(hipMemsetAsync(dL_dparam, 0, (size_t)meta->n_params * (out_dtype == NR3D_F16 ? 2 : 4), (hipStream_t)stream));
		return 0;
	}
	NR3D_CHECK(dL_dy && x && dL_dparam && workspace, "LoTD::bwd: NULL tensor pointer");
	bool handled = false;
	DparamPass p = plain_pass(meta, meta_dev, N, dL_dy, g_sn, g_se, x, dL_dparam);
	p.g_half = grad_dtype == NR3D_F16; p.out_half = out_dtype == NR3D_F16; p.assign = assign != 0;
	p.max_level = max_level;
	p.workspace = workspace; p.workspace_bytes = workspace_bytes; p.st = (hipStream_t)stream;
	p.fold = (uint32_t *)fold;
	NR3D_TRY(dparam_binned(p, handled));
	NR3D_CHECK(handled, "LoTD::bwd_dparam_typed: the pair-record path does not apply to this meta / workspace");
	return 0;
}

extern "C" int nr3d_lotd_bwd_dparam_levels(const nr3d_lotd_meta_t *meta, const void *meta_dev, uint32_t N, int x_dtype,
                                           int param_dtype, const void *dL_dy, int64_t g_sn, int64_t g_se, const void *x,
                                           const void *params, const int64_t *batch_inds, const int64_t *batch_offsets,
                                           uint32_t batch_data_size, uint32_t n_batches, int32_t min_level,
                                           int32_t max_level, void *dL_dparam, void *workspace, uint64_t workspace_bytes,
                                           void *stream) {
	if (int rc = check_common(meta, meta_dev, x_dtype, param_dtype, true)) return rc;
	NR3D_CHECK(min_level >= 0, "LoTD::bwd: min_level must be >= 0");
	DparamPass p = plain_pass(meta, meta_dev, N, dL_dy, g_sn, g_se, x, dL_dparam);
	p.params = params; p.p_half = param_dtype == NR3D_F16;
	p.batch = Batch{batch_inds, batch_offsets, batch_data_size, meta->n_params}; p.n_batches = n_batches;
	p.min_level = min_level; p.max_level = max_level;
	p.workspace = workspace; p.workspace_bytes = workspace_bytes; p.st = (hipStream_t)stream;
	return launch_bwd_dparam(p);
}

extern "C" void nr3d_lotd_set_dparam_chunk_log2(int log2_points) { set_dparam_chunk_log2(log2_points); }

extern "C" uint64_t nr3d_lotd_dparam_workspace_bytes(const nr3d_lotd_meta_t *meta, uint32_t n_points, uint32_t n_batches) {
	return dparam_workspace_bytes(meta, n_points, n_batches);
}

extern "C" int nr3d_lotd_bwd_bwd_dparam(const nr3d_lotd_meta_t *meta, const void *meta_dev, uint32_t N, int x_dtype,
                                        int param_dtype, const void *dL_ddLdx, const void *dL_dy, int64_t g_sn,
                                        int64_t g_se, const void *x, const void *params, const int64_t *batch_inds,
                                        const int64_t *batch_offsets, uint32_t batch_data_size, uint32_t n_batches,
                                        int32_t max_level, void *dL_dparam, void *workspace, uint64_t workspace_bytes,
                                        void *stream) {
	if (int rc = check_common(meta, meta_dev, x_dtype, param_dtype, true)) return rc;
	NR3D_CHECK(N == 0 || dL_ddLdx != nullptr, "LoTD::bwd_bwd_input: dL_ddLdx is NULL");
	DparamPass p = plain_pass(meta, meta_dev, N, dL_dy, g_sn, g_se, x, dL_dparam);
	p.second = true; p.dL_ddLdx = (const float *)dL_ddLdx;
	p.params = params; p.p_half = param_dtype == NR3D_F16;
	p.batch = Batch{batch_inds, batch_offsets, batch_data_size, meta->n_params}; p.n_batches = n_batches;
	p.min_level = 0; p.max_level = max_level;
	p.workspace = workspace; p.workspace_bytes = workspace_bytes; p.st = (hipStream_t)stream;
	return launch_bwd_dparam(p);
}

extern "C" int nr3d_lotd_bwd_bwd_ddLdy(const nr3d_lotd_meta_t *meta, uint32_t N, int x_dtype, int param_dtype,
                                       const void *dL_ddLdx, const void *dy_dx, int64_t d_sn, int64_t d_se,
                                       void *dL_ddLdy, int64_t o_sn, int64_t o_se, void *stream) {
	NR3D_CHECK(meta != nullptr, "LoTD: meta is NULL");
	NR3D_CHECK(x_dtype == NR3D_F32 && param_dtype == NR3D_F32, "LoTD::bwd_bwd_ddLdy: f32 only");
	if (N == 0) return 0;
	NR3D_CHECK(dL_ddLdx && dy_dx && dL_ddLdy, "LoTDEncoding::bwd_bwd_input: need `dy_dx` to compute `dL_d(dLdy)`.");
	DISPATCH_D(meta->n_dims_to_encode, {
		hipLaunchKernelGGL(k_contract_ddLdy<D>, dim3(div_up(N, kBlock), meta->n_encoded_dims), dim3(kBlock), 0,
// ... 131 lines not shown
```

nr3d_lib_amd/csrc/lotd_bin.hip:

```cpp
#include "lotd_vm.h"
#include "lotd_sorted.h"
#include <stdlib.h>
#include <type_traits>

#ifndef NR3D_BIN_LDS_KB
#define NR3D_BIN_LDS_KB 72
#define NR3D_BIN_MAX_BP 512
#endif
namespace nr3d {
namespace lotd {

constexpr int kAccThreads = 1024;
constexpr int kLdsDoubles = 16384;
constexpr int kRedSlots = 4;
#ifndef NR3D_BALLOT_RANK_BUCKETS
#define NR3D_BALLOT_RANK_BUCKETS 4
#endif
constexpr uint32_t kBallotRankBuckets = NR3D_BALLOT_RANK_BUCKETS;
constexpr int kMaxPlanLevels = 64;
constexpr uint32_t kMaxBuckets = 8192;
constexpr int kBinLdsDyn = NR3D_BIN_LDS_KB * 1024 + (int)(kMaxBuckets + 1) * 4;

#define DISPATCH_DG_BIN(D_, G_, ...)                                                 \
	do {                                                                             \
// ... 1462 lines not shown
	}
	DISPATCH_DG_BIN(D, G, {
		if (meta->c_hash_only) {
			if constexpr (D <= 3) rc = launch_class<D, G, 8, true>(p, c, pl);
			else rc = launch_class<D, G, 16, true>(p, c, pl);
		} else if (cls == 8) rc = launch_class<D, G, 8, false>(p, c, pl);
		else if (cls == 16) {
			if constexpr (D >= 3) rc = launch_class<D, G, 16, false>(p, c, pl);
		} else if (cls == 24) {
			if constexpr (D == 3) rc = launch_class<D, G, 24, false>(p, c, pl);
		} else {
			if constexpr (D == 4) rc = launch_class<D, G, 32, false>(p, c, pl);
		}
	});
	return rc;
}

int dparam_binned(const DparamPass &pass, bool &handled) {
	handled = false;
	DparamPass p = pass;
	BinLayout lay;
	const uint32_t N = p.N, nc = chunk_points(N);
	const bool forest = p.forest != nullptr;
	nr3d_lotd_meta_t narrow;
	const bool narrowed = p.workspace && stage_a_meta(p.meta, forest, narrow);
	if (narrowed) p.meta = &narrow;
	const nr3d_lotd_meta_t *meta = p.meta;
	if (!p.workspace || !binnable(meta, forest) || !layout(meta, nc, p.n_batches, lay, forest)) return 0;
	if (p.workspace_bytes < lay.total + (narrowed ? kStageAMetaBytes : 0)) return 0;
	handled = true;
	char *ws = (char *)p.workspace;
	if (narrowed) {
		k_store_meta<<<1, 256, 0, p.st>>>(narrow, (uint32_t *)(ws + lay.total));
		NR3D_HIP_CHECK(hipGetLastError());
		p.meta_dev = (const nr3d_lotd_meta_t *)(ws + lay.total);
	}
	const uint32_t D = meta->n_dims_to_encode, E = meta->n_encoded_dims;
	DparamChunk c;
	c.rec = (uint32_t *)ws;
	c.offs = (uint32_t *)(ws + lay.rec_bytes);
	c.plan_buf = (uint32_t *)(ws + lay.rec_bytes + lay.offs_bytes);
	c.partial = (float *)(ws + lay.rec_bytes + lay.offs_bytes + lay.plan_bytes);
	c.gt = (float *)(ws + lay.rec_bytes + lay.offs_bytes + lay.plan_bytes + lay.part_bytes);
	c.dev = -1;
	const bool row_major = (p.g_se == 1 && p.g_sn == (int64_t)E && E > 1) || p.g_half;
	const bool plain = !forest && p.n_batches <= 1 && !p.batch.inds && !p.batch.offsets && !p.batch.data_size;
	const bool use_pair = plain && pair_applies(meta) && !(p.second && !pair_second_enabled());
	if ((p.g_half || p.out_half) && !use_pair)
		return ::nr3d::fail("LoTD::bwd: half gradients are served natively on the pair-record path only (nr3d_lotd_half_params_ok)");
	p.assign = pass.assign && use_pair && N <= nc && p.min_level <= 0 && p.max_level >= (int32_t)meta->n_levels - 1;
	if (pass.assign && !p.assign)
		NR3D_HIP_CHECK(hipMemsetAsync(p.dparam, 0, (size_t)(p.n_batches ? p.n_batches : 1u) * meta->n_params * (p.out_half ? 2 : 4), p.st));
	if (!(N <= nc && !p.second)) p.fold = nullptr;

	for (uint32_t p0 = 0; p0 < N; p0 += nc) {
		const uint32_t n = c.n = (N - p0) < nc ? (N - p0) : nc;
		c.xc = p.x + (size_t)p0 * D;
		c.vc = p.dL_ddLdx ? p.dL_ddLdx + (size_t)p0 * D : nullptr;
		c.g_rows = p.g_half ? reinterpret_cast<const float *>(reinterpret_cast<const __half *>(p.dL_dy) + (int64_t)p0 * p.g_sn)
		                    : p.dL_dy + (int64_t)p0 * p.g_sn;
		c.gc = c.g_rows;
		c.sn = p.g_sn; c.se = p.g_se;
		c.ba = p.batch;
		if (c.ba.inds) c.ba.inds += p0;
		c.ba.first_point = p0;
		bool gt_ready = !row_major;
		auto need_gt = [&]() {
			if (gt_ready) return;
			if (p.g_half) launch_transpose<__half>(n, E, reinterpret_cast<const __half *>(c.g_rows), p.g_sn, p.g_se, c.gt, p.st);
			else launch_transpose<float>(n, E, c.g_rows, p.g_sn, p.g_se, c.gt, p.st);
			c.gc = c.gt; c.sn = 1; c.se = (int64_t)n;
			gt_ready = true;
		};
		if (use_pair) {
			need_gt();
			NR3D_TRY(pair_chunk(p, c));
			continue;
		}
		uint64_t served = 0;
		if (plain) {
			CpPlan cp;
			uint32_t max_acc = 0;
			if ((served = cp_plan(meta, n, p.min_level, p.max_level, lay.part_bytes / 4, cp, max_acc))) {
				need_gt();
				NR3D_TRY(cp_direct_route(p, c, cp, max_acc));
			}
		}
		if (!p.g_half) {
			VsPlan vsp;
			const uint64_t smask = vm_sorted_plan(meta, n, p.n_batches, forest, p.min_level, p.max_level, served, vsp);
			if (smask) {
				VsScratch vss;
				vm_sorted_scratch(vsp, n, E, p.second, forest, vss);
				if (vss.total <= lay.rec_bytes + lay.offs_bytes) {
					NR3D_TRY(vm_sorted_run(p, c, vsp, vss));
					served |= smask;
				}
			}
		}
		if (plain) {
			VmPlan vp;
			const uint64_t vmask = vm_direct_plan(meta, n, p.min_level, p.max_level, lay.part_bytes / 4, vp, served);
			if (vmask) {
				need_gt();
				NR3D_TRY(vm_direct_route(p, c, vp));
				served |= vmask;
			}
		}
		for (uint32_t cls : kClasses) {
			BinPlan pl;
			uint64_t ow;
			make_plan(meta, n, p.n_batches, cls, PlanLevels{p.min_level, p.max_level, forest, served}, pl, ow);
			if (pl.n_pseudo == 0) continue;
			need_gt();
			NR3D_TRY(class_route(p, c, pl, cls));
		}
	}
	return 0;
}

}
}
```

nr3d_lib_amd/csrc/lotd_device.h:

```cpp
#pragma once
#include "common.h"
#include <type_traits>

namespace nr3d {
namespace lotd {

constexpr int kBlock = 256;
constexpr uint32_t kPrimes[7] = {1u, 2654435761u, 805459861u, 3674653429u, 2097192037u, 1434869437u, 2165219737u};

constexpr int kSchedSegs = 16;
struct Sched {
	uint32_t n_chunks, n_pseudo, mode, n_slots;
	uint64_t skip;
	uint32_t seg_cum[8][kSchedSegs + 1];
	uint32_t seg_begin[8][kSchedSegs];
	uint32_t seg_q[8][kSchedSegs];
};

__device__ __forceinline__ bool decode_block_raw(const Sched &s, uint32_t b, uint32_t &q, uint32_t &chunk);
__device__ __forceinline__ bool decode_block(const Sched &s, uint32_t b, uint32_t &q, uint32_t &chunk) {
	if (!decode_block_raw(s, b, q, chunk)) return false;
	return s.mode == 3 || q >= 64u || !((s.skip >> q) & 1ull);
}
__device__ __forceinline__ bool decode_block_raw(const Sched &s, uint32_t b, uint32_t &q, uint32_t &chunk) {
// ... 578 lines not shown
}

__device__ __forceinline__ bool resolve(const ForestDev &fo, const Batch &ba, const Lvl &L, const Block &b,
                                        const uint32_t (&p)[3], uint32_t (&pl)[3], uint32_t &offset) {
	uint32_t owner = 0xFFFFFFFFu;
	if (!resolve_block(fo, L, b.k, p, pl, owner)) return false;
	offset = (owner == 0xFFFFFFFFu) ? b.offset : (ba.offsets ? (uint32_t)ba.offsets[owner] : owner * ba.n_params);
	return true;
}

__device__ __forceinline__ void locate_forest(const float (&xp)[3], const Lvl &L, bool smooth, Cell<3> &c) {
#pragma unroll
	for (int d = 0; d < 3; ++d) {
		const float sc = (float)L.res[d];
		const float v = __fmaf_rn(xp[d], sc, 0.5f);
		const float fl = floorf(v);
		const float t = v - fl;
		c.sc[d] = sc;
		c.g[d] = (uint32_t)fl;
		if (!smooth) {
			c.w[d] = t; c.dw[d] = 1.0f; c.ddw[d] = 0.0f;
		} else {
			c.w[d] = t * t * __fmaf_rn(-2.0f, t, 3.0f);
			c.dw[d] = 6.0f * t * (1.0f - t);
			c.ddw[d] = __fmaf_rn(-12.0f, t, 6.0f);
		}
	}
}

uint64_t dparam_workspace_bytes(const nr3d_lotd_meta_t *m, uint32_t n_points, uint32_t n_batches, bool forest = false);
void set_dparam_chunk_log2(int lg);
struct DparamPass {
	bool second;
	const nr3d_lotd_meta_t *meta, *meta_dev;
	uint32_t N;
	const float *dL_ddLdx;
	const float *dL_dy;
	int64_t g_sn, g_se;
	bool g_half;
	const float *x;
	const void *params;
	bool p_half;
	Batch batch;
	uint32_t n_batches;
	int32_t min_level, max_level;
	float *dparam;
	bool out_half;
	bool assign;
	void *workspace;
	uint64_t workspace_bytes;
	hipStream_t st;
	const ForestDev *forest;
	uint32_t *fold;
};
struct DparamChunk {
	uint32_t n;
	const float *xc, *vc;
	const float *g_rows;
	const float *gc;
	int64_t sn, se;
	Batch ba;
	uint32_t *rec, *offs, *plan_buf;
	float *partial, *gt;
	int dev;
};

template <typename F> static inline void with_bool(bool b, F &&f) { if (b) f(std::true_type{}); else f(std::false_type{}); }
template <typename F> static inline void with_tables(const void *params, bool p_half, F &&f) {
	if (p_half) f((const __half *)params); else f((const float *)params);
}
template <typename P> using pointee_t = std::remove_const_t<std::remove_pointer_t<P>>;

static inline DparamPass plain_pass(const nr3d_lotd_meta_t *meta, const void *meta_dev, uint32_t N, const void *dL_dy, int64_t g_sn,
                                    int64_t g_se, const void *x, void *dparam) {
	DparamPass p;
	p.second = false; p.meta = meta; p.meta_dev = (const nr3d_lotd_meta_t *)meta_dev; p.N = N;
	p.dL_ddLdx = nullptr; p.dL_dy = (const float *)dL_dy; p.g_sn = g_sn; p.g_se = g_se; p.g_half = false;
	p.x = (const float *)x; p.params = nullptr; p.p_half = false;
	p.batch = Batch{nullptr, nullptr, 0u, meta->n_params}; p.n_batches = 1u;
	p.min_level = 0; p.max_level = 0x7fffffff;
	p.dparam = (float *)dparam; p.out_half = false; p.assign = false;
	p.workspace = nullptr; p.workspace_bytes = 0; p.st = nullptr;
	p.forest = nullptr; p.fold = nullptr;
	return p;
}

int dparam_binned(const DparamPass &pass, bool &handled);
bool dparam_one_pass(uint32_t n_points);

bool pair_applies(const nr3d_lotd_meta_t *m);
uint32_t pair_direct_levels(const nr3d_lotd_meta_t *m, uint32_t n_points);
void pair_layout(const nr3d_lotd_meta_t *m, uint32_t n_chunk, uint64_t &rec_bytes, uint64_t &offs_bytes, uint64_t &plan_bytes,
                 uint64_t &part_bytes);
int pair_chunk(const DparamPass &p, DparamChunk &c);
uint64_t pair_fold_layout(const nr3d_lotd_meta_t *m, uint32_t n, int32_t max_level, uint32_t &gcols, uint32_t &zero_words,
                          uint32_t &slot_off);

}
}
```

nr3d_lib_amd/csrc/lotd_pair.hip:

```cpp
#include "lotd_device.h"
#include <stdlib.h>


namespace nr3d {
namespace lotd {

constexpr uint32_t kPEpbMax = 8192;
constexpr int kPAccThreads = 1024;
constexpr int kPLdsMax = 2 * (int)kPEpbMax;
constexpr int kPMaxLv = 32;
constexpr uint32_t kPMaxNb = 511;
typedef uint32_t u32x4 __attribute__((ext_vector_type(4)));

struct PairPlan {
	uint32_t qmap[kPMaxLv];
	uint32_t nb[kPMaxLv];
	uint32_t epb[kPMaxLv];
	uint32_t shift[kPMaxLv];
	uint32_t bucket_base[kPMaxLv + 1];
	uint32_t offs_base[kPMaxLv];
	uint32_t n_blk, n_pseudo;
	uint32_t cap;
	uint32_t lg;
	uint32_t sum_log2;
};

constexpr uint32_t kDirectNb = 4, kDirectMaxLv = 8, kDirectMaxWg = 640;
struct DirectPlan {
	uint32_t n;
	uint32_t qmap[kDirectMaxLv], nb[kDirectMaxLv], epb[kDirectMaxLv], shift[kDirectMaxLv];
	uint32_t bucket_base[kDirectMaxLv + 1];
	uint32_t lg, sum_log2, R, pts_per_rep;
	uint32_t merge_min;
};


constexpr uint32_t kPairBp = 1024, kPairLg = 12, kPairUnroll = 4, kDirectRotate = 8, kPairUnits = 1536;
static bool pair_quad_enabled() { return opt::on(NR3D_OPT_PAIR_QUAD); }
static uint32_t pair_fixed() { return opt::on(NR3D_OPT_PAIR_FIXED) ? 1u : 0u; }

__device__ __forceinline__ float pair_wp2(float wp, float Cm, float Em, float &Cuse) {
	const float floor_c = fmaxf(1e-18f * fabsf(Em), 1e-30f);
	Cuse = !(fabsf(Cm) < floor_c) ? Cm : copysignf(floor_c, Cm);
	return __fmaf_rn(Em, __builtin_amdgcn_rcpf(Cuse), wp);
}
template <bool SECOND = false>
__device__ __forceinline__ void pair_records(const Lvl &L, uint32_t sh, uint32_t epb, uint32_t lg, const float (&xp)[3], float g0,
                                             float g1, bool smooth, uint32_t (&hdr)[4], uint32_t (&bkt)[4], float (&A)[4][2],
                                             float (&wpm)[SECOND ? 4 : 1], uint32_t (&cell)[3], uint32_t nb, bool &valid,
                                             const float *__restrict__ vin, uint32_t &qmask, float &wy, bool quad_on) {
	Cell<3> c;
	locate<3>(xp, L, smooth, c);
	valid = true;
	float a[3] = {0.0f, 0.0f, 0.0f};
	if constexpr (SECOND) {
#pragma unroll
		for (int d = 0; d < 3; ++d) a[d] = c.sc[d] * vin[d] * c.dw[d];
	}
	if constexpr (!SECOND) { qmask = 0; wy = c.w[1]; }
	if (L.type == NR3D_LOD_Dense) {
		const float wp = c.w[2];
#pragma unroll
		for (uint32_t m = 0; m < 4; ++m) {
			const uint32_t bx = m & 1u, by = m >> 1;
			const uint32_t row = (c.g[0] + bx) * L.res[1] + (c.g[1] + by);
			const uint32_t e0 = row * L.res[2] + c.g[2];
			const uint32_t b = row >> sh;
			const uint32_t i0 = e0 - b * epb;
			valid = valid && b < nb && c.g[2] + 1u < L.res[2];
			bkt[m] = b;
			hdr[m] = i0 | ((i0 + 1u) << 13);
			const float wx = bx ? c.w[0] : 1.0f - c.w[0], wy = by ? c.w[1] : 1.0f - c.w[1];
			const float wo = wx * wy;
			if constexpr (!SECOND) { A[m][0] = g0 * wo; A[m][1] = g1 * wo; wpm[0] = wp; }
			else {
				const float Cm = __fmaf_rn(bx ? a[0] : -a[0], wy, (by ? a[1] : -a[1]) * wx);
				float Cuse;
				wpm[m] = pair_wp2(wp, Cm, a[2] * wo, Cuse);
				A[m][0] = g0 * Cuse; A[m][1] = g1 * Cuse;
			}
		}
		if constexpr (!SECOND) {
#pragma unroll
			for (uint32_t bx = 0; bx < 2; ++bx)
				if (quad_on && bkt[bx] == bkt[bx + 2u] && (hdr[bx] & 8191u) + L.res[2] + 1u < 8192u) qmask |= 1u << bx;
		}
	} else {
		const float wp = c.w[0];
		const bool pow2 = (L.size & (L.size - 1u)) == 0u;
		const uint32_t emask = (1u << lg) - 1u;
#pragma unroll
		for (uint32_t m = 0; m < 4; ++m) {
			const uint32_t by = m & 1u, bz = m >> 1;
			const uint32_t K = ((c.g[1] + by) * kPrimes[1]) ^ ((c.g[2] + bz) * kPrimes[2]);
			const uint32_t h0 = c.g[0] ^ K, h1 = (c.g[0] + 1u) ^ K;
			const uint32_t e0 = pow2 ? (h0 & (L.size - 1u)) : (h0 % L.size);
			const uint32_t e1 = pow2 ? (h1 & (L.size - 1u)) : (h1 % L.size);
			bkt[m] = e0 >> lg;
			valid = valid && (e1 >> lg) == bkt[m] && bkt[m] < nb;
			hdr[m] = (e0 & emask) | ((e1 & emask) << 13);
			const float wy = by ? c.w[1] : 1.0f - c.w[1], wz = bz ? c.w[2] : 1.0f - c.w[2];
			const float wo = wy * wz;
			if constexpr (!SECOND) { A[m][0] = g0 * wo; A[m][1] = g1 * wo; wpm[0] = wp; }
			else {
				const float Cm = __fmaf_rn(by ? a[1] : -a[1], wz, (bz ? a[2] : -a[2]) * wy);
				float Cuse;
				wpm[m] = pair_wp2(wp, Cm, a[0] * wo, Cuse);
				A[m][0] = g0 * Cuse; A[m][1] = g1 * Cuse;
			}
		}
	}
#pragma unroll
	for (int d = 0; d < 3; ++d) cell[d] = c.g[d];
}

__device__ __forceinline__ void pair_buckets(const Lvl &L, uint32_t sh, uint32_t lg, const float (&xp)[3], bool smooth, uint32_t (&bkt)[4]) {
	Cell<3> c;
	locate<3>(xp, L, smooth, c);
	if (L.type == NR3D_LOD_Dense) {
#pragma unroll
		for (uint32_t m = 0; m < 4; ++m) bkt[m] = ((c.g[0] + (m & 1u)) * L.res[1] + (c.g[1] + (m >> 1))) >> sh;
	} else {
		const bool pow2 = (L.size & (L.size - 1u)) == 0u;
#pragma unroll
		for (uint32_t m = 0; m < 4; ++m) {
			const uint32_t h0 = c.g[0] ^ ((c.g[1] + (m & 1u)) * kPrimes[1]) ^ ((c.g[2] + (m >> 1)) * kPrimes[2]);
			bkt[m] = (pow2 ? (h0 & (L.size - 1u)) : (h0 % L.size)) >> lg;
		}
	}
}

template <int kPBP, bool SECOND = false>
__device__ __forceinline__ void pair_level(const PairPlan &plan, uint32_t ql, const Lvl &L, bool active, const float (&xp)[3],
                                           float g0, float g1, uint32_t smooth, u32x4 *__restrict__ stage,
                                           uint32_t *__restrict__ hist, uint32_t *__restrict__ zero_next, uint32_t *scan_lds,
                                           u32x4 *__restrict__ dst, uint32_t *__restrict__ ob, uint32_t ob_stride,
                                           const float *__restrict__ vin = nullptr, bool quad_on = false) {
	const uint32_t nb = plan.nb[ql];
	const uint32_t lane = threadIdx.x & 63u;
	uint32_t hdr[4], bkt[4], cell[3] = {0xFFFFFFFFu, 0xFFFFFFFFu, 0xFFFFFFFFu};
	constexpr int kW = SECOND ? 3 : 0;
	constexpr bool QUADS = !SECOND;
	uint32_t qmask = 0;
	float wy = 0.0f;
	float A[4][2], wp[SECOND ? 4 : 1];
#pragma unroll
	for (int m = 0; m < 4; ++m) { hdr[m] = 0; bkt[m] = 0; A[m][0] = 0.0f; A[m][1] = 0.0f; wp[m & kW] = 0.0f; }
	if (zero_next)
		for (uint32_t b = threadIdx.x; b <= kPMaxNb; b += kPBP) zero_next[b] = 0;
	if (active) {
		bool valid;
		pair_records<SECOND>(L, plan.shift[ql], plan.epb[ql], plan.lg, xp, g0, g1, smooth != 0, hdr, bkt, A, wp, cell, nb, valid, vin, qmask, wy,
		                     quad_on);
		active = valid;
	}

	bool emit = active, split = false;
	float Hh[4][2];
#pragma unroll
	for (int m = 0; m < 4; ++m) { Hh[m][0] = 0.0f; Hh[m][1] = 0.0f; }
	{
		auto prev = [](uint32_t v) { return (uint32_t)__builtin_amdgcn_update_dpp(0, (int)v, 0x138, 0xf, 0xf, false); };
		bool same = active && lane > 0;
#pragma unroll
		for (int d = 0; d < 3; ++d) same = same && (prev(cell[d]) == cell[d]);
		same = same && (prev((uint32_t)active) != 0u);
		const unsigned long long cont = __ballot(same);
		if (__popcll(cont) >= 16) {
			float lo[4][2], hi[4][2];
#pragma unroll
			for (int m = 0; m < 4; ++m)
#pragma unroll
				for (int f = 0; f < 2; ++f) { lo[m][f] = (1.0f - wp[m & kW]) * A[m][f]; hi[m][f] = wp[m & kW] * A[m][f]; }
#pragma unroll
			for (int off = 1; off < 64; off <<= 1) {
				const unsigned long long need = (1ull << off) - 1ull;
				const bool take = (lane + off < 64) && (((cont >> (lane + 1)) & need) == need);
#pragma unroll
				for (int m = 0; m < 4; ++m)
#pragma unroll
					for (int f = 0; f < 2; ++f) {
						const float tl = __shfl_down(lo[m][f], off, 64), th = __shfl_down(hi[m][f], off, 64);
						if (take) { lo[m][f] += tl; hi[m][f] += th; }
					}
			}
			const bool head_multi = active && !same && lane < 63 && ((cont >> (lane + 1)) & 1ull);
			if (same) emit = false;
			if (head_multi) {
// ... 7 lines not shown
	}

	uint32_t rank[4] = {0, 0, 0, 0};
	const uint32_t cnt = emit ? (split ? 2u : 1u) : 0u;
	auto emits = [&](int m) {
		if constexpr (QUADS) return emit && !(!split && m >= 2 && ((qmask >> (m - 2)) & 1u));
		else return emit;
	};
	if (nb <= 4) {
#pragma unroll
		for (int m = 0; m < 4; ++m) {
			const bool e_m = emits(m);
			const uint32_t bv = e_m ? bkt[m] : 0xFFFFFFFFu;
			unsigned long long todo = __ballot(e_m);
			while (todo) {
				const int leader = __ffsll((long long)todo) - 1;
				const uint32_t v = (uint32_t)__builtin_amdgcn_readlane((int)bv, leader);
				const bool mine = e_m && bv == v;
				const unsigned long long m1 = __ballot(mine), m2 = __ballot(mine && split);
				uint32_t first = 0;
				if ((int)lane == leader) first = atomicAdd(&hist[v], (uint32_t)(__popcll(m1) + __popcll(m2)));
				first = (uint32_t)__builtin_amdgcn_readlane((int)first, leader);
				const unsigned long long below = (1ull << lane) - 1ull;
				if (mine) rank[m] = first + (uint32_t)(__popcll(m1 & below) + __popcll(m2 & below));
				todo &= ~m1;
			}
		}
	} else {
#pragma unroll
		for (int m = 0; m < 4; ++m) {
			const bool e_m = emits(m);
			const uint32_t bv = e_m ? bkt[m] : 0xFFFFFFFFu;
			const unsigned long long em = __ballot(e_m);
			bool done = !e_m;
			if (em) {
				const int leader = __ffsll((long long)em) - 1;
				const uint32_t v = (uint32_t)__builtin_amdgcn_readlane((int)bv, leader);
				const bool mine = e_m && bv == v;
				const unsigned long long m1 = __ballot(mine);
				if (__popcll(m1) >= 8) {
					const unsigned long long m2 = __ballot(mine && split);
					uint32_t first = 0;
					if ((int)lane == leader) first = atomicAdd(&hist[v], (uint32_t)(__popcll(m1) + __popcll(m2)));
					first = (uint32_t)__builtin_amdgcn_readlane((int)first, leader);
					const unsigned long long below = (1ull << lane) - 1ull;
					if (mine) { rank[m] = first + (uint32_t)(__popcll(m1 & below) + __popcll(m2 & below)); done = true; }
				}
			}
			if (!done) rank[m] = atomicAdd(&hist[bv], cnt);
		}
	}
	__syncthreads();

	{
		const uint32_t b = threadIdx.x;
		const uint32_t v = (b < nb) ? hist[b] : 0u;
		uint32_t inc = v;
#pragma unroll
		for (int off = 1; off < 64; off <<= 1) {
			const uint32_t t = __shfl_up(inc, off, 64);
			if ((int)lane >= off) inc += t;
		}
		if (lane == 63) scan_lds[threadIdx.x >> 6] = inc;
		__syncthreads();
		uint32_t wave_off = 0;
#pragma unroll
		for (int k = 0; k < kPBP / 64; ++k) { const uint32_t t = scan_lds[k]; if (k < (int)(threadIdx.x >> 6)) wave_off += t; }
		if (b <= nb) hist[b] = wave_off + inc - v;
		__syncthreads();
	}

	if (emit) {
#pragma unroll
		for (int m = 0; m < 4; ++m) {
			if constexpr (QUADS) { if (!emits(m)) continue; }
			const uint32_t pos = hist[bkt[m]] + rank[m];
			if (QUADS && !split && m < 2 && ((qmask >> m) & 1u)) {
				const uint32_t wzq = (uint32_t)__float2uint_rn(wp[0] * 16777215.0f), wyq = (uint32_t)__float2uint_rn(wy * 16777215.0f);
				stage[pos] = u32x4{(hdr[m] & 8191u) | (((wyq >> 8) & 8191u) << 13) | (4u << 26) | ((wyq >> 21) << 29),
				                   wzq | ((wyq & 255u) << 24), __float_as_uint(A[m][0] + A[m + 2][0]), __float_as_uint(A[m][1] + A[m + 2][1])};
			} else if (!split) {
				stage[pos] = u32x4{hdr[m] | (3u << 26), __float_as_uint(wp[m & kW]), __float_as_uint(A[m][0]), __float_as_uint(A[m][1])};
			} else {
				stage[pos] = u32x4{(hdr[m] & 0x1FFFu) | (1u << 26), 0u, __float_as_uint(A[m][0]), __float_as_uint(A[m][1])};
				stage[pos + 1] = u32x4{(hdr[m] & 0x3FFE000u) | (2u << 26), 0u, __float_as_uint(Hh[m][0]), __float_as_uint(Hh[m][1])};
			}
		}
	}
	__syncthreads();

	const uint32_t total = hist[nb];
	for (uint32_t v = threadIdx.x; v < total; v += kPBP) __builtin_nontemporal_store(stage[v], dst + v);
	for (uint32_t b = threadIdx.x; b <= nb; b += kPBP) ob[(size_t)b * ob_stride] = hist[b];
	if (zero_next) __syncthreads();
}

template <int kPBP>
__device__ __forceinline__ void pair_gmax(uint32_t gbits, uint32_t *scan_lds, uint32_t *__restrict__ gmax) {
	const uint32_t lane = threadIdx.x & 63u;
#pragma unroll
	for (int off = 32; off >= 1; off >>= 1) gbits = max(gbits, (uint32_t)__shfl_xor((int)gbits, off, 64));
	__syncthreads();
	if (lane == 0) scan_lds[threadIdx.x >> 6] = gbits;
	__syncthreads();
	if (threadIdx.x == 0) {
		uint32_t m = 0;
#pragma unroll
		for (int k = 0; k < kPBP / 64; ++k) m = max(m, scan_lds[k]);
		if (m > __hip_atomic_load(gmax, __ATOMIC_RELAXED, __HIP_MEMORY_SCOPE_AGENT)) atomicMax(gmax, m);
	}
}

template <int kPBP, bool SECOND = false>
__global__ __launch_bounds__(kPBP, kPBP == 768 ? 6 : 8)  void k_pair_bin(PairPlan plan, const nr3d_lotd_meta_t *__restrict__ md, uint32_t n,
                                                   int32_t max_level, uint32_t smooth, const float *__restrict__ x,
                                                   const float *__restrict__ g, int64_t g_sn, int64_t g_se,
                                                   u32x4 *__restrict__ rec, uint32_t *__restrict__ offs_g,
                                                   uint32_t *__restrict__ gmax, DirectPlan dp, const float *__restrict__ vin_,
                                                   uint32_t quad_on) {
	constexpr uint32_t kPCap = (uint32_t)kPBP * 4u;
	extern __shared__ __attribute__((aligned(16))) uint32_t smem[];
	__shared__ uint32_t scan_lds[kPBP / 64];
	u32x4 *stage = reinterpret_cast<u32x4 *>(smem);
	uint32_t *hist = smem + (size_t)kPCap * 4;
	const uint32_t blk = blockIdx.x, ql = blockIdx.y;
	const uint32_t q = plan.qmap[ql], nb = plan.nb[ql];
	const uint32_t level = meta_level_of(md, q);
	const Lvl L = load_level(md, level);
	const uint32_t i = blk * kPBP + threadIdx.x;
	for (uint32_t b = threadIdx.x; b <= nb; b += kPBP) hist[b] = 0;
	__syncthreads();
	const bool active = (i < n) && ((int32_t)level <= max_level);
	float xp[3] = {0.0f, 0.0f, 0.0f}, vin[3] = {0.0f, 0.0f, 0.0f}, g0 = 0.0f, g1 = 0.0f;
	if (active) {
#pragma unroll
		for (int d = 0; d < 3; ++d) xp[d] = x[(size_t)i * 3 + d];
		g0 = g[(int64_t)i * g_sn + (int64_t)(q * 2) * g_se];
		g1 = g[(int64_t)i * g_sn + (int64_t)(q * 2 + 1) * g_se];
		if constexpr (SECOND) {
#pragma unroll
			for (int d = 0; d < 3; ++d) vin[d] = vin_[(size_t)i * 3 + d];
		}
	}
	pair_level<kPBP, SECOND>(plan, ql, L, active, xp, g0, g1, smooth, stage, hist, nullptr, scan_lds,
	                         rec + ((size_t)ql * plan.n_blk + blk) * (size_t)plan.cap, offs_g + plan.offs_base[ql] + blk, plan.n_blk, vin,
	                         quad_on != 0u);
	if (gmax) {
		uint32_t gbits;
		if constexpr (!SECOND) {
			gbits = max(__float_as_uint(g0) & 0x7FFFFFFFu, __float_as_uint(g1) & 0x7FFFFFFFu);
			if (ql == 0 && i < n)
				for (uint32_t e = 0; e < dp.n; ++e) {
					const uint32_t qd = dp.qmap[e];
					if ((int32_t)meta_level_of(md, qd) > max_level) continue;
					gbits = max(gbits, __float_as_uint(g[(int64_t)i * g_sn + (int64_t)(qd * 2) * g_se]) & 0x7FFFFFFFu);
					gbits = max(gbits, __float_as_uint(g[(int64_t)i * g_sn + (int64_t)(qd * 2 + 1) * g_se]) & 0x7FFFFFFFu);
				}
		} else {
			auto bound = [&](const Lvl &Lq, float ga, float gb) {
				const float m = __uint_as_float(max(__float_as_uint(ga) & 0x7FFFFFFFu, __float_as_uint(gb) & 0x7FFFFFFFu)) * 1.5f *
				                ((float)(Lq.res[0] - 2u) * fabsf(vin[0]) + (float)(Lq.res[1] - 2u) * fabsf(vin[1]) + (float)(Lq.res[2] - 2u) * fabsf(vin[2]));
				return __float_as_uint(m) & 0x7FFFFFFFu;
			};
			gbits = bound(L, g0, g1);
			if (ql == 0 && i < n) {
				if (!active) {
#pragma unroll
					for (int d = 0; d < 3; ++d) vin[d] = vin_[(size_t)i * 3 + d];
				}
				for (uint32_t e = 0; e < dp.n; ++e) {
					const uint32_t qd = dp.qmap[e];
					if ((int32_t)meta_level_of(md, qd) > max_level) continue;
					const Lvl Ld = load_level(md, meta_level_of(md, qd));
					gbits = max(gbits, bound(Ld, g[(int64_t)i * g_sn + (int64_t)(qd * 2) * g_se], g[(int64_t)i * g_sn + (int64_t)(qd * 2 + 1) * g_se]));
				}
			}
		}
		pair_gmax<kPBP>(gbits, scan_lds, gmax);
	}
}

__device__ __forceinline__ uint32_t gmax_slots(const uint32_t *__restrict__ slots, uint32_t n_slots, uint32_t *red) {
	uint32_t m = 0;
	for (uint32_t k = threadIdx.x; k < n_slots; k += 1024u) m = max(m, slots[k]);
#pragma unroll
	for (int off = 32; off >= 1; off >>= 1) m = max(m, (uint32_t)__shfl_xor((int)m, off, 64));
	__syncthreads();
	if ((threadIdx.x & 63u) == 0) red[threadIdx.x >> 6] = m;
	__syncthreads();
	m = 0;
#pragma unroll
	for (int k = 0; k < 16; ++k) m = max(m, red[k]);
	__syncthreads();
	return m;
}

__device__ __forceinline__ void pair_plan_block(const PairPlan &plan, const uint32_t *__restrict__ offs_g, uint32_t n_units,
                                                uint32_t *__restrict__ tot, uint32_t *__restrict__ rep,
                                                uint32_t *__restrict__ item_start, uint32_t *__restrict__ ticket, uint32_t bid,
                                                uint32_t nblk, const uint32_t *__restrict__ slots, uint32_t n_slots,
                                                uint32_t *__restrict__ gmax_out, bool empty_one) {
	__shared__ uint64_t red[16];
	__shared__ uint64_t carry_s;
	__shared__ uint32_t last_s;
	const uint32_t lane = threadIdx.x & 63, wave = threadIdx.x >> 6;
	const uint32_t NB = plan.bucket_base[plan.n_pseudo];
	{
		const uint32_t fb = bid * 16 + wave;
		if (fb < NB) {
			uint32_t q = 0;
			while (q + 1 < plan.n_pseudo && plan.bucket_base[q + 1] <= fb) ++q;
			const uint32_t *ob0 = offs_g + plan.offs_base[q] + (size_t)(fb - plan.bucket_base[q]) * plan.n_blk;
			const uint32_t *ob1 = ob0 + plan.n_blk;
			uint32_t sum = 0;
			for (uint32_t blk = lane; blk < plan.n_blk; blk += 64) sum += ob1[blk] - ob0[blk];
#pragma unroll
			for (int off = 32; off >= 1; off >>= 1) sum += __shfl_xor(sum, off, 64);
			if (lane == 0) __hip_atomic_store(tot + fb, sum, __ATOMIC_RELAXED, __HIP_MEMORY_SCOPE_AGENT);
		}
	}
	__syncthreads();
	if (threadIdx.x == 0) {
		__builtin_amdgcn_fence(__ATOMIC_RELEASE, "agent");
		asm volatile("s_waitcnt vmcnt(0)" ::: "memory");
		last_s = (atomicAdd(ticket, 1u) == nblk - 1u) ? 1u : 0u;
		__builtin_amdgcn_fence(__ATOMIC_ACQUIRE, "agent");
	}
	__syncthreads();
	if (!last_s) return;
	if (slots) {
		const uint32_t gb = gmax_slots(slots, n_slots, reinterpret_cast<uint32_t *>(red));
		if (threadIdx.x == 0) gmax_out[0] = gb;
	}
	auto ld_tot = [&](uint32_t fb) { return (uint64_t)__hip_atomic_load(tot + fb, __ATOMIC_RELAXED, __HIP_MEMORY_SCOPE_AGENT); };
	uint64_t part = 0;
	for (uint32_t fb = threadIdx.x; fb < NB; fb += 1024) part += ld_tot(fb);
#pragma unroll
	for (int off = 32; off >= 1; off >>= 1) part += __shfl_xor(part, off, 64);
	if (lane == 0) red[wave] = part;
	__syncthreads();
	uint64_t total = 0;
#pragma unroll
	for (int w = 0; w < 16; ++w) total += red[w];
	const uint64_t unit = total / n_units > 0 ? total / n_units : 1;
	if (threadIdx.x == 0) carry_s = 0;
	__syncthreads();
	for (uint32_t base = 0; base < NB; base += 1024) {
		const uint32_t fb = base + threadIdx.x;
		uint32_t r = 0;
		if (fb < NB) {
			const uint64_t t = ld_tot(fb);
			r = t == 0 ? (empty_one ? 1u : 0u) : (uint32_t)((t + unit / 2) / unit);
			if (t != 0 && r < 1) r = 1;
			if (r > plan.n_blk) r = plan.n_blk;
			rep[fb] = r;
		}
		uint64_t inc = r;
#pragma unroll
		for (int off = 1; off < 64; off <<= 1) { const uint64_t t2 = __shfl_up(inc, off, 64); if ((int)lane >= off) inc += t2; }
		__syncthreads();
		if (lane == 63) red[wave] = inc;
		__syncthreads();
		uint64_t woff = 0, tsum = 0;
#pragma unroll
		for (int w = 0; w < 16; ++w) { if (w < (int)wave) woff += red[w]; tsum += red[w]; }
		const uint64_t c = carry_s;
		if (fb < NB) item_start[fb] = (uint32_t)(c + woff + inc - r);
		__syncthreads();
// ... 66 lines not shown
	const uint32_t b = fb - dp.bucket_base[e], q = dp.qmap[e];
	const Lvl L = load_level(md, meta_level_of(md, q));
	const uint32_t foff0 = meta_cnt_of(md, q) * 2u, kPLds = 2u << dp.lg;
	if (t >= kPLds) return;
	float *p = pair_target(L, dp.epb[e], dp.lg, foff0, b, t, dparam, half_out);
	if (!p) return;
	const float sum = pair_replica_sum(dpart + (size_t)fb * dp.R * kPLds + t, dp.R, kPLds);
	pair_st(p, (assign ? 0.0f : pair_ld(p, half_out)) + sum, half_out);
}

template <int kUnroll, bool FIX>
__global__ __launch_bounds__(kPAccThreads, 8)  void k_pair_accum(PairPlan plan, const nr3d_lotd_meta_t *__restrict__ md,
                                                             const u32x4 *__restrict__ rec,
                                                             const uint32_t *__restrict__ offs_g,
                                                             const uint32_t *__restrict__ rep_g,
                                                             const uint32_t *__restrict__ item_start,
                                                             const uint32_t *__restrict__ gmax,
                                                             float *__restrict__ partial, float *__restrict__ dparam,
                                                             uint32_t out_half, uint32_t *__restrict__ bticket, uint32_t n_dred,
                                                             DirectPlan dp, const float *__restrict__ dpart) {
	extern __shared__ __attribute__((aligned(16))) unsigned long long acc_raw[];
	__shared__ uint32_t last_s;
	if (blockIdx.x < n_dred) {
		const uint32_t rows = (2u << dp.lg) / kPAccThreads;
		pair_direct_sum(dp, md, dpart, dparam, out_half, blockIdx.x / rows, (blockIdx.x % rows) * kPAccThreads + threadIdx.x);
		return;
	}
	const uint32_t item = blockIdx.x - n_dred;
	double *acc = reinterpret_cast<double *>(acc_raw);
	const uint32_t NB = plan.bucket_base[plan.n_pseudo];
	const cu32_t istart = (cu32_t)item_start, irep = (cu32_t)rep_g;
	if (item >= istart[NB]) return;
	uint32_t lo = 0, hi = NB;
	while (hi - lo > 1) { const uint32_t mid = (lo + hi) >> 1; if (istart[mid] <= item) lo = mid; else hi = mid; }
	const uint32_t fb = lo, R = irep[fb], r = item - istart[fb];
	uint32_t q = 0;
	while (q + 1 < plan.n_pseudo && plan.bucket_base[q + 1] <= fb) ++q;
	const uint32_t b = fb - plan.bucket_base[q];
	const uint32_t qg = plan.qmap[q];
	const Lvl L = load_level(md, meta_level_of(md, qg));
	const uint32_t foff0 = meta_cnt_of(md, qg) * 2u, epb = plan.epb[q];
	PairFix fx = {1.0, 1.0, false};
	if constexpr (FIX) fx = pair_fix(gmax, plan.sum_log2);
	const bool fix = FIX && fx.on;

	const uint32_t kPEpb = 1u << plan.lg, kPLds = 2u << plan.lg;
	for (uint32_t t = threadIdx.x; t < kPLds; t += kPAccThreads) acc_raw[t] = 0ull;
	__syncthreads();

	const uint32_t lane = threadIdx.x & 63, wave = threadIdx.x >> 6;
	constexpr uint32_t n_waves = kPAccThreads / 64;
	const uint32_t blk_lo = 0u, blk_hi = (plan.n_blk > r) ? (plan.n_blk - r + R - 1u) / R : 0u;
	const uint32_t *ob0 = offs_g + plan.offs_base[q] + (size_t)b * plan.n_blk;
	const uint32_t *ob1 = ob0 + plan.n_blk;
	const uint32_t kPCap = plan.cap;
	const u32x4 *rec_q = rec + (size_t)q * plan.n_blk * (size_t)kPCap;
	const uint32_t per_wave = (blk_hi - blk_lo + n_waves - 1) / n_waves;
	const uint32_t w_lo = min(blk_lo + wave * per_wave, blk_hi), w_hi = min(w_lo + per_wave, blk_hi);
	constexpr int kGroup = 8;
	for (uint32_t blk0 = w_lo; blk0 < w_hi; blk0 += 64) {
		const uint32_t mb = blk0 + lane;
		const uint32_t s_l = (mb < w_hi) ? ob0[r + R * mb] : 0u;
		const uint32_t e_l = (mb < w_hi) ? ob1[r + R * mb] : 0u;
		const uint32_t n_run = min(64u, w_hi - blk0);
		const u32x4 *rec_b = rec_q + (size_t)(r + R * blk0) * kPCap;
		for (uint32_t j0 = 0; j0 < n_run; j0 += kGroup) {
			uint32_t pre[kGroup + 1], rbase[kGroup];
			pre[0] = 0;
#pragma unroll
			for (int u = 0; u < kGroup; ++u) {
				const uint32_t j = min(j0 + (uint32_t)u, 63u);
				const uint32_t s_j = __builtin_amdgcn_readlane(s_l, j), e_j = __builtin_amdgcn_readlane(e_l, j);
				const uint32_t nrec = (j0 + (uint32_t)u < n_run) ? e_j - s_j : 0u;
				rbase[u] = s_j + j * R * kPCap - pre[u];
				pre[u + 1] = pre[u] + nrec;
			}
			const uint32_t total = pre[kGroup];
			for (uint32_t p0 = 0; p0 < total; p0 += 64u * kUnroll) {
				u32x4 rv[kUnroll];
#pragma unroll
				for (int v = 0; v < kUnroll; ++v) {
					const uint32_t pos = p0 + 64u * (uint32_t)v + lane;
					uint32_t at = rbase[0];
#pragma unroll
					for (int u = 1; u < kGroup; ++u) at = (pos >= pre[u]) ? rbase[u] : at;
					rv[v] = __builtin_nontemporal_load(rec_b + (size_t)(pos < total ? at + pos : rbase[0]));
				}
#pragma unroll
				for (int v = 0; v < kUnroll; ++v)
					if (p0 + 64u * (uint32_t)v + lane < total) {
						const uint32_t h = rv[v].x, fl = (h >> 26) & 7u;
						const uint32_t i0 = h & 8191u, i1 = (h >> 13) & 8191u;
						const float w = __uint_as_float(rv[v].y), a0 = __uint_as_float(rv[v].z), a1 = __uint_as_float(rv[v].w);
						if (fl == 4u) {
							const uint32_t wyq = (((h >> 13) & 8191u) << 8) | (rv[v].y >> 24) | ((h >> 29) << 21), wzq = rv[v].y & 0xFFFFFFu;
							const float wy = (float)wyq * (1.0f / 16777215.0f), wz = (float)wzq * (1.0f / 16777215.0f);
							const float q00 = (1.0f - wy) * (1.0f - wz), q01 = (1.0f - wy) * wz, q10 = wy * (1.0f - wz), q11 = wy * wz;
							const uint32_t i2 = i0 + L.res[2];
							if (fix) {
								atomicAdd(&acc_raw[i0], to_fix(q00 * a0, fx.scale)); atomicAdd(&acc_raw[kPEpb + i0], to_fix(q00 * a1, fx.scale));
								atomicAdd(&acc_raw[i0 + 1u], to_fix(q01 * a0, fx.scale)); atomicAdd(&acc_raw[kPEpb + i0 + 1u], to_fix(q01 * a1, fx.scale));
								atomicAdd(&acc_raw[i2], to_fix(q10 * a0, fx.scale)); atomicAdd(&acc_raw[kPEpb + i2], to_fix(q10 * a1, fx.scale));
								atomicAdd(&acc_raw[i2 + 1u], to_fix(q11 * a0, fx.scale)); atomicAdd(&acc_raw[kPEpb + i2 + 1u], to_fix(q11 * a1, fx.scale));
							} else {
								atomicAdd(&acc[i0], (double)(q00 * a0)); atomicAdd(&acc[kPEpb + i0], (double)(q00 * a1));
								atomicAdd(&acc[i0 + 1u], (double)(q01 * a0)); atomicAdd(&acc[kPEpb + i0 + 1u], (double)(q01 * a1));
								atomicAdd(&acc[i2], (double)(q10 * a0)); atomicAdd(&acc[kPEpb + i2], (double)(q10 * a1));
								atomicAdd(&acc[i2 + 1u], (double)(q11 * a0)); atomicAdd(&acc[kPEpb + i2 + 1u], (double)(q11 * a1));
							}
							continue;
						}
						const bool pair = fl == 3u;
						const float wl = pair ? 1.0f - w : 1.0f, wh = pair ? w : 1.0f;
						if (fix) {
							if (fl & 1u) { atomicAdd(&acc_raw[i0], to_fix(wl * a0, fx.scale)); atomicAdd(&acc_raw[kPEpb + i0], to_fix(wl * a1, fx.scale)); }
							if (fl & 2u) { atomicAdd(&acc_raw[i1], to_fix(wh * a0, fx.scale)); atomicAdd(&acc_raw[kPEpb + i1], to_fix(wh * a1, fx.scale)); }
// ... 40 lines not shown
		float *p[kFlush];
		float v[kFlush], old[kFlush];
#pragma unroll
		for (int k = 0; k < kFlush; ++k) {
			const uint32_t t = tb + (uint32_t)k * kPAccThreads;
			p[k] = (t < kPLds) ? pair_target(L, epb, plan.lg, foff0, b, t, dparam, (out_half & 1u) != 0) : nullptr;
			v[k] = p[k] ? value(t) : 0.0f;
		}
		const bool half_out = (out_half & 1u) != 0, assign = (out_half & 2u) != 0;
#pragma unroll
		for (int k = 0; k < kFlush; ++k) old[k] = (p[k] && !assign) ? pair_ld(p[k], half_out) : 0.0f;
#pragma unroll
		for (int k = 0; k < kFlush; ++k) if (p[k]) pair_st(p[k], old[k] + v[k], half_out);
	}
}

template <bool FIX, bool SECOND = false>
__global__ __launch_bounds__(kPAccThreads, 8) void k_pair_direct(DirectPlan dp, const nr3d_lotd_meta_t *__restrict__ md, uint32_t n,
                                                                 int32_t max_level, uint32_t smooth, const float *__restrict__ x,
                                                                 const float *__restrict__ g, int64_t g_sn, int64_t g_se,
                                                                 const uint32_t *__restrict__ gmax, float *__restrict__ partial,
                                                                 const float *__restrict__ vin_, uint32_t plan_rows, PairPlan plan,
                                                                 const uint32_t *__restrict__ offs_g, uint32_t n_units,
                                                                 uint32_t *__restrict__ tot, uint32_t *__restrict__ rep,
                                                                 uint32_t *__restrict__ item_start, uint32_t *__restrict__ ticket,
                                                                 const uint32_t *__restrict__ slots, uint32_t n_slots,
                                                                 uint32_t *__restrict__ gmax_out, uint32_t empty_one) {
	extern __shared__ __attribute__((aligned(16))) unsigned long long acc_raw[];
	__shared__ uint32_t queue[kPAccThreads / 64][128];
	if (blockIdx.y >= gridDim.y - plan_rows) {
		const uint32_t bid = (blockIdx.y - (gridDim.y - plan_rows)) * gridDim.x + blockIdx.x, nblk = (plan.bucket_base[plan.n_pseudo] + 15u) / 16u;
		if (bid < nblk) pair_plan_block(plan, offs_g, n_units, tot, rep, item_start, ticket, bid, nblk, slots, n_slots, gmax_out, empty_one != 0u);
		return;
	}
	double *acc = reinterpret_cast<double *>(acc_raw);
	const uint32_t r = blockIdx.x, fb = blockIdx.y;
	uint32_t e = 0;
	while (e + 1 < dp.n && dp.bucket_base[e + 1] <= fb) ++e;
	const uint32_t b = fb - dp.bucket_base[e], q = dp.qmap[e];
	const uint32_t level = meta_level_of(md, q);
	const Lvl L = load_level(md, level);
	const uint32_t kPEpb = 1u << dp.lg, kPLds = 2u << dp.lg;
	PairFix fx = {1.0, 1.0, false};
	if constexpr (FIX) fx = slots ? pair_fix_bits(gmax_slots(slots, n_slots, &queue[0][0]), dp.sum_log2) : pair_fix(gmax, dp.sum_log2);
	const bool fix = FIX && fx.on;
	for (uint32_t t = threadIdx.x; t < kPLds; t += kPAccThreads) acc_raw[t] = 0ull;
	__syncthreads();
	if ((int32_t)level <= max_level) {
		const uint32_t p_lo = r * dp.pts_per_rep;
		auto process = [&](uint32_t i) {
			float xp[3];
#pragma unroll
			for (int d = 0; d < 3; ++d) xp[d] = x[(size_t)i * 3 + d];
			const float g0 = g[(int64_t)i * g_sn + (int64_t)(q * 2) * g_se], g1 = g[(int64_t)i * g_sn + (int64_t)(q * 2 + 1) * g_se];
			uint32_t hdr[4], bkt[4], cell[3];
			constexpr int kW = SECOND ? 3 : 0;
			float A[4][2], wp[SECOND ? 4 : 1], vin[3] = {0.0f, 0.0f, 0.0f};
			bool valid;
			if constexpr (SECOND) {
#pragma unroll
				for (int d = 0; d < 3; ++d) vin[d] = vin_[(size_t)i * 3 + d];
			}
			uint32_t qmask;
			float wy_unused;
			pair_records<SECOND>(L, dp.shift[e], dp.epb[e], dp.lg, xp, g0, g1, smooth != 0, hdr, bkt, A, wp, cell, dp.nb[e], valid, vin, qmask, wy_unused, false);
			float lo[4][2], hi[4][2];
#pragma unroll
			for (int m = 0; m < 4; ++m)
#pragma unroll
				for (int f = 0; f < 2; ++f) { lo[m][f] = (1.0f - wp[m & kW]) * A[m][f]; hi[m][f] = wp[m & kW] * A[m][f]; }
			bool rotate = false;
			{
				const uint32_t ln = threadIdx.x & 63u;
				auto prev = [](uint32_t v) { return (uint32_t)__builtin_amdgcn_update_dpp(0, (int)v, 0x138, 0xf, 0xf, false); };
				bool same = ln > 0;
#pragma unroll
				for (int d = 0; d < 3; ++d) same = same && (prev(cell[d]) == cell[d]);
				same = same && (prev(1u) != 0u);
				rotate = (uint32_t)__popcll(__ballot(same)) >= dp.merge_min;
			}
			if (!valid) return;
			if (rotate) {
				const uint32_t ln = threadIdx.x & 63u;
				const bool sw = (ln & 4u) != 0u, fs = (ln & 8u) != 0u;
#pragma unroll
				for (uint32_t step = 0; step < 4u; ++step) {
					const uint32_t m = (step + ln) & 3u;
					auto sel = [&](auto a0, auto a1, auto a2, auto a3) { return m == 0u ? a0 : (m == 1u ? a1 : (m == 2u ? a2 : a3)); };
					if (sel(bkt[0], bkt[1], bkt[2], bkt[3]) != b) continue;
					const uint32_t hd = sel(hdr[0], hdr[1], hdr[2], hdr[3]);
					const float l0 = sel(lo[0][0], lo[1][0], lo[2][0], lo[3][0]), l1 = sel(lo[0][1], lo[1][1], lo[2][1], lo[3][1]);
					const float h0 = sel(hi[0][0], hi[1][0], hi[2][0], hi[3][0]), h1 = sel(hi[0][1], hi[1][1], hi[2][1], hi[3][1]);
					const uint32_t i0 = hd & 8191u, i1 = (hd >> 13) & 8191u;
					const uint32_t ea = sw ? i1 : i0, eb = sw ? i0 : i1;
					const float a0 = sw ? h0 : l0, a1 = sw ? h1 : l1, b0 = sw ? l0 : h0, b1 = sw ? l1 : h1;
					const uint32_t fa = fs ? kPEpb : 0u, fb2 = fs ? 0u : kPEpb;
					if (fix) {
						atomicAdd(&acc_raw[fa + ea], to_fix(fs ? a1 : a0, fx.scale)); atomicAdd(&acc_raw[fb2 + ea], to_fix(fs ? a0 : a1, fx.scale));
						atomicAdd(&acc_raw[fa + eb], to_fix(fs ? b1 : b0, fx.scale)); atomicAdd(&acc_raw[fb2 + eb], to_fix(fs ? b0 : b1, fx.scale));
					} else {
						atomicAdd(&acc[fa + ea], (double)(fs ? a1 : a0)); atomicAdd(&acc[fb2 + ea], (double)(fs ? a0 : a1));
						atomicAdd(&acc[fa + eb], (double)(fs ? b1 : b0)); atomicAdd(&acc[fb2 + eb], (double)(fs ? b0 : b1));
					}
				}
				return;
			}
#pragma unroll
// ... 90 lines not shown
	if (blockIdx.x >= NB) {
		const uint32_t fb = (blockIdx.x - NB) / kRedRows, sub = (blockIdx.x - NB) % kRedRows;
		pair_direct_sum(dp, md, dpart, dparam, out_half, fb, (blockIdx.y * kRedRows + sub) * kPAccThreads + threadIdx.x);
		return;
	}
	const uint32_t fb = blockIdx.x;
	const uint32_t R = rep_g[fb];
	if (R == 1 || (R == 0 && !assign)) return;
	uint32_t q = 0;
	while (q + 1 < plan.n_pseudo && plan.bucket_base[q + 1] <= fb) ++q;
	const uint32_t b = fb - plan.bucket_base[q], qg = plan.qmap[q];
	const Lvl L = load_level(md, meta_level_of(md, qg));
	const uint32_t foff0 = meta_cnt_of(md, qg) * 2u;
	const uint32_t kPLds = 2u << plan.lg;
	const float *part0 = partial + (size_t)item_start[fb] * kPLds;
	for (uint32_t row = 0; row < kRedRows; ++row) {
		const uint32_t t = (blockIdx.y * kRedRows + row) * kPAccThreads + threadIdx.x;
		if (t >= kPLds) return;
		float *p = pair_target(L, plan.epb[q], plan.lg, foff0, b, t, dparam, half_out);
		if (!p) continue;
		const float sum = pair_replica_sum(part0 + t, R, kPLds);
		pair_st(p, (assign ? 0.0f : pair_ld(p, half_out)) + sum, half_out);
	}
}

static bool pair_enabled() { return opt::on(NR3D_OPT_LOTD_PAIR); }

bool pair_applies(const nr3d_lotd_meta_t *m) {
	if (!pair_enabled()) return false;
	if (!m || m->n_dims_to_encode != 3 || m->n_feat_per_pseudo_lvl != 2 || !m->c_hash_only) return false;
	if (m->n_pseudo_levels > (uint32_t)kPMaxLv) return false;
	for (uint32_t l = 0; l < m->n_levels; ++l) {
		const nr3d_lotd_level_t &L = m->levels[l];
		const uint32_t kPEpb = 1u << kPairLg;
		if (L.type == NR3D_LOD_Dense) {
			if (L.res[2] > kPEpb) return false;
			const uint64_t rows = (uint64_t)L.res[0] * L.res[1];
			uint32_t lg = 0;
			while ((2ull << lg) * L.res[2] <= kPEpb) ++lg;
			if (((rows + (1ull << lg) - 1) >> lg) > kPMaxNb) return false;
		} else if (L.type == NR3D_LOD_Hash) {
			if (L.size <= kPEpb) continue;
			if ((L.size & (L.size - 1u)) != 0u || L.res[0] > kPEpb) return false;
			if ((L.size >> kPairLg) > kPMaxNb) return false;
		} else {
			return false;
		}
	}
	return true;
}


static void pair_plan(const nr3d_lotd_meta_t *m, uint32_t n_chunk, int32_t min_level, int32_t max_level, PairPlan &plan,
                      uint64_t &offs_words, uint64_t skip_pseudo = 0) {
	plan.n_blk = div_up(n_chunk, kPairBp);
	plan.cap = kPairBp * 4u;
	plan.lg = kPairLg;
	plan.sum_log2 = 3;
	while ((1ull << (plan.sum_log2 - 3)) < n_chunk) ++plan.sum_log2;
	const uint32_t kPEpb = 1u << plan.lg;
	uint32_t nq = 0;
	uint64_t base = 0;
	for (uint32_t q = 0; q < m->n_pseudo_levels; ++q) {
		const int32_t lv = (int32_t)m->map_levels[q];
		if (lv < min_level || lv > max_level || ((skip_pseudo >> q) & 1ull)) continue;
		const nr3d_lotd_level_t &L = m->levels[lv];
		uint32_t nb, epb, sh;
		if (L.type == NR3D_LOD_Dense) {
			sh = 0;
			while ((2ull << sh) * L.res[2] <= kPEpb) ++sh;
			epb = (1u << sh) * L.res[2];
			nb = (uint32_t)((((uint64_t)L.res[0] * L.res[1]) + (1ull << sh) - 1) >> sh);
		} else {
			sh = plan.lg; epb = kPEpb;
			nb = L.size <= kPEpb ? 1u : (L.size >> plan.lg);
		}
		plan.qmap[nq] = q; plan.nb[nq] = nb; plan.epb[nq] = epb; plan.shift[nq] = sh;
		plan.bucket_base[nq] = nq ? plan.bucket_base[nq - 1] + plan.nb[nq - 1] : 0u;
		plan.offs_base[nq] = (uint32_t)base;
		base += (uint64_t)(nb + 1) * plan.n_blk;
		++nq;
	}
	plan.n_pseudo = nq;
	plan.bucket_base[nq] = nq ? plan.bucket_base[nq - 1] + plan.nb[nq - 1] : 0u;
	offs_words = base;
}

static bool pair_direct_enabled() { return opt::on(NR3D_OPT_PAIR_DIRECT); }
static uint64_t pair_direct_plan(const PairPlan &full, uint32_t n, DirectPlan &dp) {
	dp.n = 0; dp.lg = full.lg; dp.sum_log2 = full.sum_log2; dp.R = 1; dp.pts_per_rep = n;
	dp.merge_min = kDirectRotate;
	dp.bucket_base[0] = 0;
	if (!pair_direct_enabled()) return 0;
	uint64_t mask = 0;
	for (uint32_t ql = 0; ql < full.n_pseudo && dp.n < kDirectMaxLv; ++ql) {
		if (full.nb[ql] > kDirectNb || full.qmap[ql] >= 64u) continue;
		if (dp.bucket_base[dp.n] + full.nb[ql] > kDirectMaxWg) break;
		const uint32_t e = dp.n++;
		dp.qmap[e] = full.qmap[ql]; dp.nb[e] = full.nb[ql]; dp.epb[e] = full.epb[ql]; dp.shift[e] = full.shift[ql];
		dp.bucket_base[e + 1] = dp.bucket_base[e] + full.nb[ql];
		mask |= 1ull << full.qmap[ql];
	}
	if (dp.n == 0 || dp.n == full.n_pseudo) { dp.n = 0; return 0; }
	const uint32_t nbk = dp.bucket_base[dp.n];
	uint32_t R = kDirectMaxWg / nbk;
	R = R > 128u ? 128u : R;
	const uint32_t by_points = div_up(n, 2048u);
	R = R > by_points ? by_points : R;
	dp.R = R < 1u ? 1u : R;
	dp.pts_per_rep = div_up(n, dp.R);
	return mask;
}

uint32_t pair_direct_levels(const nr3d_lotd_meta_t *m, uint32_t n_points) {
	PairPlan plan;
	uint64_t ow;
	pair_plan(m, n_points, 0, 0x7fffffff, plan, ow);
	DirectPlan dp;
	pair_direct_plan(plan, n_points, dp);
	return dp.n;
}

void pair_layout(const nr3d_lotd_meta_t *m, uint32_t n_chunk, uint64_t &rec_bytes, uint64_t &offs_bytes, uint64_t &plan_bytes,
                 uint64_t &part_bytes) {
	PairPlan plan;
	uint64_t ow;
	pair_plan(m, n_chunk, 0, 0x7fffffff, plan, ow);
	const uint32_t NB = plan.bucket_base[plan.n_pseudo];
	rec_bytes = (uint64_t)plan.n_pseudo * plan.n_blk * plan.cap * 16;
	offs_bytes = ((ow * 4 + 255) / 256) * 256;
	plan_bytes = (((uint64_t)NB * 3 + 4) * 4 + 255) / 256 * 256;
	part_bytes = (uint64_t)(kPairUnits + NB + kDirectMaxWg) * (2u << plan.lg) * 4;
}

void launch_plan_items(uint32_t NB, uint32_t n_blk, uint32_t units, const uint32_t *tot, uint32_t *rep, uint32_t *item_start,
                       hipStream_t st);

constexpr uint32_t kFoldHead = 64;
uint64_t pair_fold_layout(const nr3d_lotd_meta_t *m, uint32_t n, int32_t max_level, uint32_t &gcols, uint32_t &zero_words,
                          uint32_t &slot_off) {
	gcols = zero_words = slot_off = 0;
	if (!opt::on(NR3D_OPT_PAIR_FOLD) || !m || !pair_applies(m) || n == 0 || max_level < 0 || !dparam_one_pass(n)) return 0;
	if (2u * m->n_pseudo_levels != m->n_encoded_dims) return 0;
	uint32_t nq = 0;
	while (nq < m->n_pseudo_levels && (int32_t)m->map_levels[nq] <= max_level) ++nq;
	for (uint32_t q = nq; q < m->n_pseudo_levels; ++q)
		if ((int32_t)m->map_levels[q] <= max_level) return 0;
	if (nq == 0) return 0;
	PairPlan pl;
	uint64_t ow;
	pair_plan(m, n, 0, max_level, pl, ow);
	gcols = 2u * nq;
	zero_words = kFoldHead + pl.bucket_base[pl.n_pseudo];
	slot_off = (zero_words + 63u) & ~63u;
	return (uint64_t)(slot_off + div_up(n, (uint32_t)kBlock)) * 4u;
}

int pair_chunk(const DparamPass &p, DparamChunk &c) {
	const nr3d_lotd_meta_t *meta = p.meta, *md = p.meta_dev;
	const uint32_t n = c.n, units = kPairUnits;
	const uint32_t out_flags = (p.out_half ? 1u : 0u) | (p.assign ? 2u : 0u);
	const int32_t min_level = p.min_level, max_level = p.max_level;
	const float *x = c.xc, *g = c.gc, *vin = p.second ? c.vc : nullptr;
	const int64_t g_sn = c.sn, g_se = c.se;
	uint32_t *offs = c.offs, *plan_buf = c.plan_buf, *fold = p.fold;
	float *dparam = p.dparam, *partial = c.partial;
	hipStream_t st = p.st;
	uint32_t f_gcols = 0, f_zero = 0, f_slot = 0;
	if (fold && (vin || min_level > 0 || pair_fold_layout(meta, n, max_level, f_gcols, f_zero, f_slot) == 0)) fold = nullptr;
	const uint32_t *slots = fold ? fold + f_slot : nullptr;
	const uint32_t n_slots = div_up(n, (uint32_t)kBlock);
	PairPlan pl;
	uint64_t ow;
	pair_plan(meta, n, min_level, max_level, pl, ow);
	if (pl.n_pseudo == 0) return 0;
	DirectPlan dp;
	dp.n = 0;
	const uint32_t NB_full = pl.bucket_base[pl.n_pseudo];
	{
		const uint64_t skip = pair_direct_plan(pl, n, dp);
		if (skip) pair_plan(meta, n, min_level, max_level, pl, ow, skip);
	}
	uint32_t nb_max = 0;
	for (uint32_t q = 0; q < pl.n_pseudo; ++q) nb_max = nb_max > pl.nb[q] ? nb_max : pl.nb[q];
	const uint32_t NB = pl.bucket_base[pl.n_pseudo];
	uint32_t *tot = plan_buf, *rep = plan_buf + NB, *item_start = plan_buf + 2 * (size_t)NB;
	uint32_t *gmax = fold ? fold : plan_buf + 3 * (size_t)NB + 2;
	uint32_t *bticket = fold ? fold + kFoldHead : nullptr;
	const size_t bin_lds_max = (size_t)kPairBp * 4 * 16 + (size_t)(kPMaxNb + 2) * 8;
	static LdsOnce once_bin, once_acc;
	NR3D_TRY(NR3D_LDS_LIMIT(once_bin, c.dev, (int)bin_lds_max, k_pair_bin<kPairBp>, k_pair_bin<kPairBp, true>));
	NR3D_TRY(NR3D_LDS_LIMIT(once_acc, c.dev, kPLdsMax * 8, k_pair_direct<true>, k_pair_direct<false>, k_pair_direct<true, true>,
	                        k_pair_direct<false, true>, k_pair_accum<kPairUnroll, false>, k_pair_accum<kPairUnroll, true>));
	if (!fold) NR3D_HIP_CHECK(hipMemsetAsync(gmax, 0, 2 * sizeof(uint32_t), st));
	const size_t bin_lds = (size_t)kPairBp * 4 * 16 + (size_t)(nb_max + 1) * 4;
	const uint32_t quad_on = (!vin && pair_quad_enabled()) ? 1u : 0u;
#define NR3D_PAIR_BIN(BP) if (vin) NR3D_PAIR_BIN_(BP, true); else NR3D_PAIR_BIN_(BP, false)
#define NR3D_PAIR_BIN_(BP, SEC) hipLaunchKernelGGL((k_pair_bin<BP, SEC>), dim3(pl.n_blk, pl.n_pseudo), dim3(BP), bin_lds, st, pl, md, n, max_level, \
	meta->interpolation_type, x, g, g_sn, g_se, (u32x4 *)c.rec, offs, fold ? nullptr : gmax, dp, vin, quad_on)
	{
		prof::Scope ps(NR3D_PROF_LOTD_BIN, st);
		NR3D_PAIR_BIN(kPairBp);
	}
#undef NR3D_PAIR_BIN
#undef NR3D_PAIR_BIN_
	float *dpart = partial + (size_t)(units + NB_full) * (2u << pl.lg);
	const uint32_t nbk_direct = dp.n ? dp.bucket_base[dp.n] : 0u;
	const bool plan_in_direct = fold && dp.n && pl.n_pseudo;
	const uint32_t plan_rows = plan_in_direct ? div_up(div_up(NB, 16u), dp.R) : 0u;
	const uint32_t empty_one = (fold && (out_flags & 2u)) ? 1u : 0u;
	if (dp.n) {
		prof::Scope ps(NR3D_PROF_LOTD_DIRECT, st);
		auto direct = [&](auto kern) {
			hipLaunchKernelGGL(kern, dim3(dp.R, nbk_direct + plan_rows), dim3(kPAccThreads), (size_t)(16u << pl.lg), st, dp, md, n, max_level,
			                   meta->interpolation_type, x, g, g_sn, g_se, gmax, dpart, vin, plan_rows, pl, offs, units, tot, rep, item_start,
			                   gmax + 1, slots, n_slots, fold, empty_one);
		};
		if (vin) { if (pair_fixed()) direct(k_pair_direct<true, true>); else direct(k_pair_direct<false, true>); }
		else     { if (pair_fixed()) direct(k_pair_direct<true, false>); else direct(k_pair_direct<false, false>); }
	}
	if (pl.n_pseudo == 0) {
		if (dp.n)
			hipLaunchKernelGGL(k_pair_direct_reduce, dim3(nbk_direct, (2u << pl.lg) / kPAccThreads), dim3(kPAccThreads), 0, st, dp, md, dpart,
			                   dparam, out_flags);
		NR3D_LAUNCH_CHECK();
		return 0;
	}
	if (!plan_in_direct)
		hipLaunchKernelGGL(k_pair_plan, dim3(div_up(NB, 16)), dim3(1024), 0, st, pl, offs, units, tot, rep, item_start, gmax + 1, slots, n_slots,
		                   fold, empty_one);
	const uint32_t n_dred = fold ? nbk_direct * ((2u << pl.lg) / kPAccThreads) : 0u;
#define NR3D_PAIR_ACC(U, F) hipLaunchKernelGGL((k_pair_accum<U, F>), dim3(n_dred + units + NB), dim3(kPAccThreads), (size_t)(16u << pl.lg), st, pl, md, \
	(const u32x4 *)c.rec, offs, rep, item_start, gmax, partial, dparam, out_flags, bticket, n_dred, dp, dpart)
	{
		prof::Scope ps(NR3D_PROF_LOTD_ACCUM, st);
		if (pair_fixed()) NR3D_PAIR_ACC(kPairUnroll, true); else NR3D_PAIR_ACC(kPairUnroll, false);
	}
#undef NR3D_PAIR_ACC
	if (!fold)
		hipLaunchKernelGGL(k_pair_reduce, dim3(NB + nbk_direct * kRedRows, div_up((2u << pl.lg) / kPAccThreads, kRedRows)), dim3(kPAccThreads), 0, st, pl, md, rep,
		                   item_start, partial, dparam, out_flags, NB, dp, dpart);
	NR3D_LAUNCH_CHECK();
	return 0;
}

}
}
```

Before: 1151 Mpoints/s.

## Read row-major dL_dy in pair binning and transpose only direct levels

The contract_dx kernel no longer writes a full feature-major transpose of dL_dy. It now writes only the rows needed by the direct-accumulation levels, and the pair-bin kernel reads gradients straight from the row-major [N,E] buffer. The offset array is packed into start/count 16-bit fields, and record capacity is now per pseudo-level with an alignment padding option (default 8). The aim is to cut transpose write traffic and offset reads, at the cost of more LDS in the bin kernel and strided gradient reads.

```diff
diff --git a/include/nr3d_hip.h b/include/nr3d_hip.h
--- a/include/nr3d_hip.h
+++ b/include/nr3d_hip.h
@@ -8,7 +8,7 @@
 
 enum { NR3D_F32 = 0, NR3D_F16 = 1, NR3D_F64 = 2, NR3D_I32 = 3, NR3D_I64 = 4, NR3D_U8 = 5, NR3D_I16 = 6, NR3D_I8 = 7 };
 
-#define NR3D_ABI_VERSION 16
+#define NR3D_ABI_VERSION 17
 
 const char *nr3d_last_error(void);
 int nr3d_abi_version(void);
@@ -50,7 +50,9 @@
 	NR3D_OPT_VM_SORTED = 18,
 	NR3D_OPT_MLP_X3 = 19,
 	NR3D_OPT_PAIR_FOLD = 20,
-	NR3D_OPT_COUNT = 21
+	NR3D_OPT_PAIR_ROWMAJOR = 21,
+	NR3D_OPT_PAIR_ALIGN = 22,
+	NR3D_OPT_COUNT = 23
 };
 int nr3d_set_option(int id, int64_t value);
 int64_t nr3d_get_option(int id);
@@ -104,6 +106,7 @@
                      const void *dL_dy, int64_t dldy_sn, int64_t dldy_se,
                      const void *dy_dx, int64_t dydx_sn, int64_t dydx_se, void *dL_dx,
                      void *dL_dy_T ,
+                     int dL_dy_T_direct ,
                      int32_t max_level, void *fold ,
                      void *stream);
 
@@ -131,7 +134,8 @@
 int nr3d_lotd_bwd_dparam_typed(const nr3d_lotd_meta_t *meta, const void *meta_dev, uint32_t n_points, int grad_dtype,
                                const void *dL_dy, int64_t g_sn, int64_t g_se, const void *x, int32_t max_level,
                                int out_dtype, int assign, void *dL_dparam, void *workspace, uint64_t workspace_bytes,
-                               void *fold, void *stream);
+                               void *fold, const void *dL_dy_T_direct, void *stream);
+int nr3d_lotd_pair_rowmajor_ok(const nr3d_lotd_meta_t *meta, uint32_t n_points);
 uint64_t nr3d_lotd_pair_fold_bytes(const nr3d_lotd_meta_t *meta, uint32_t n_points, int32_t max_level);
 
 int nr3d_lotd_bwd_bwd_ddLdy(const nr3d_lotd_meta_t *meta, uint32_t n_points, int x_dtype, int param_dtype,
diff --git a/nr3d_lib_amd/_abi.py b/nr3d_lib_amd/_abi.py
--- a/nr3d_lib_amd/_abi.py
+++ b/nr3d_lib_amd/_abi.py
@@ -1,4 +1,4 @@
-ABI_VERSION = 16
+ABI_VERSION = 17
 SIGNATURES = {
     'nr3d_abi_version': ('int', []),
     'nr3d_alpha_to_vw_backward': ('int', ['uint32_t', 'uint64_t', 'ptr', 'ptr', 'ptr', 'ptr', 'float', 'float', 'ptr', 'ptr']),
@@ -19,8 +19,8 @@
     'nr3d_lotd_bwd_bwd_dx_workspace_bytes': ('uint64_t', ['ptr', 'uint32_t']),
     'nr3d_lotd_bwd_dparam': ('int', ['ptr', 'ptr', 'uint32_t', 'int', 'int', 'ptr', 'int64_t', 'int64_t', 'ptr', 'ptr', 'ptr', 'ptr', 'uint32_t', 'uint32_t', 'int32_t', 'ptr', 'ptr', 'uint64_t', 'ptr']),
     'nr3d_lotd_bwd_dparam_levels': ('int', ['ptr', 'ptr', 'uint32_t', 'int', 'int', 'ptr', 'int64_t', 'int64_t', 'ptr', 'ptr', 'ptr', 'ptr', 'uint32_t', 'uint32_t', 'int32_t', 'int32_t', 'ptr', 'ptr', 'uint64_t', 'ptr']),
-    'nr3d_lotd_bwd_dparam_typed': ('int', ['ptr', 'ptr', 'uint32_t', 'int', 'ptr', 'int64_t', 'int64_t', 'ptr', 'int32_t', 'int', 'int', 'ptr', 'ptr', 'uint64_t', 'ptr', 'ptr']),
-    'nr3d_lotd_bwd_dx': ('int', ['ptr', 'uint32_t', 'int', 'int', 'ptr', 'int64_t', 'int64_t', 'ptr', 'int64_t', 'int64_t', 'ptr', 'ptr', 'int32_t', 'ptr', 'ptr']),
+    'nr3d_lotd_bwd_dparam_typed': ('int', ['ptr', 'ptr', 'uint32_t', 'int', 'ptr', 'int64_t', 'int64_t', 'ptr', 'int32_t', 'int', 'int', 'ptr', 'ptr', 'uint64_t', 'ptr', 'ptr', 'ptr']),
+    'nr3d_lotd_bwd_dx': ('int', ['ptr', 'uint32_t', 'int', 'int', 'ptr', 'int64_t', 'int64_t', 'ptr', 'int64_t', 'int64_t', 'ptr', 'ptr', 'int', 'int32_t', 'ptr', 'ptr']),
     'nr3d_lotd_dLdy_feature_major': ('int', ['uint32_t', 'uint32_t', 'int', 'ptr', 'int64_t', 'int64_t', 'ptr', 'ptr']),
     'nr3d_lotd_dparam_workspace_bytes': ('uint64_t', ['ptr', 'uint32_t', 'uint32_t']),
     'nr3d_lotd_forest_bwd_bwd_dx': ('int', ['ptr', 'ptr', 'ptr', 'uint32_t', 'ptr', 'ptr', 'ptr', 'ptr', 'int', 'ptr', 'ptr', 'uint32_t', 'int32_t', 'ptr', 'ptr']),
@@ -36,6 +36,7 @@
     'nr3d_lotd_pair_direct_levels': ('int', ['ptr', 'uint32_t']),
     'nr3d_lotd_pair_fold_bytes': ('uint64_t', ['ptr', 'uint32_t', 'int32_t']),
     'nr3d_lotd_pair_path_ok': ('int', ['ptr']),
+    'nr3d_lotd_pair_rowmajor_ok': ('int', ['ptr', 'uint32_t']),
     'nr3d_lotd_set_dparam_chunk_log2': ('void', ['int']),
     'nr3d_march_composite_bwd': ('int', ['uint32_t', 'ptr', 'ptr', 'ptr', 'ptr', 'ptr', 'float', 'float', 'int', 'ptr', 'ptr', 'ptr', 'ptr', 'ptr', 'ptr', 'ptr', 'ptr', 'ptr', 'ptr', 'uint64_t', 'ptr', 'ptr']),
     'nr3d_march_composite_fwd': ('int', ['uint32_t', 'ptr', 'ptr', 'ptr', 'ptr', 'ptr', 'ptr', 'ptr', 'int', 'float', 'float', 'float', 'uint32_t', 'ptr', 'ptr', 'ptr', 'ptr', 'ptr', 'ptr', 'uint64_t', 'uint64_t', 'ptr', 'ptr', 'ptr', 'ptr', 'ptr', 'ptr', 'ptr', 'ptr', 'uint64_t', 'ptr', 'float', 'float', 'int', 'ptr', 'ptr', 'ptr', 'ptr', 'ptr', 'ptr']),
diff --git a/nr3d_lib_amd/_hip.py b/nr3d_lib_amd/_hip.py
--- a/nr3d_lib_amd/_hip.py
+++ b/nr3d_lib_amd/_hip.py
@@ -129,7 +129,8 @@
 
 OPTION_IDS = dict(lotd_pair=0, pair_quad=1, pair_second=2, pair_direct=3, pair_fixed=4, fwd_pairlane=5, fwd_split=6,
                   fwd_lds_stage=7, hvp_levels=8, hvp_pairlane=9, hvp_split=10, vm_split=11, cp_direct=12, march_group=13,
-                  pack_scan=14, sort_wave=15, vm_direct=16, direct_fixed=17, vm_sorted=18, mlp_x3=19, pair_fold=20)
+                  pack_scan=14, sort_wave=15, vm_direct=16, direct_fixed=17, vm_sorted=18, mlp_x3=19, pair_fold=20,
+                  pair_rowmajor=21, pair_align=22)
 
 
 def set_option(name, value):
diff --git a/nr3d_lib_amd/bindings/_forest.py b/nr3d_lib_amd/bindings/_forest.py
--- a/nr3d_lib_amd/bindings/_forest.py
+++ b/nr3d_lib_amd/bindings/_forest.py
@@ -144,7 +144,7 @@
         if need_input_grad:
             j, jsn, jse = _lotd._jac_view(dy_dx.detach(), N, E, 3)
             H.check(H.lib().nr3d_lotd_bwd_dx(
-                C.byref(m._cmeta()), N, H.F32, H.F32, H.ptr(g32), E, 1, H.ptr(j), jsn, jse, H.ptr(dL_dx), None, max_level, None,
+                C.byref(m._cmeta()), N, H.F32, H.F32, H.ptr(g32), E, 1, H.ptr(j), jsn, jse, H.ptr(dL_dx), None, 0, max_level, None,
                 st))
         if need_param_grad:
             x32, (p32, pcode) = _lotd._f32c(input.detach()), _lotd._ptab(params)
diff --git a/nr3d_lib_amd/bindings/_lotd.py b/nr3d_lib_amd/bindings/_lotd.py
--- a/nr3d_lib_amd/bindings/_lotd.py
+++ b/nr3d_lib_amd/bindings/_lotd.py
@@ -373,26 +373,31 @@
         st = H.stream_of(input)
         tag = ("dx" if need_input_grad else "") + ("dp" if need_param_grad else "")
         with _Prof(m, f"LoTD{D}-bwd-{tag}", N):
-            gT = fold = None
+            gT = gT_direct = fold = None
             if need_input_grad and N > 0:
                 j, jsn, jse = _jac_view(dy_dx.detach(), N, E, D)
                 if (need_param_grad and not batched and USE_BINNED_DPARAM and gse == 1 and gsn == E
                         and g32.data_ptr() % 16 == 0):
-                    gT = H.empty((E, N), dtype=torch.float32, device=dev)
+                    if typed and not native and H.lib().nr3d_lotd_pair_rowmajor_ok(C.byref(m._cmeta()), N):
+                        n_dir = int(H.lib().nr3d_lotd_pair_direct_levels(C.byref(m._cmeta()), N))
+                        gT_direct = H.empty((max(2 * n_dir, 1), N), dtype=torch.float32, device=dev)
+                    else:
+                        gT = H.empty((E, N), dtype=torch.float32, device=dev)
                     if typed:
                         nfold = H.lib().nr3d_lotd_pair_fold_bytes(C.byref(m._cmeta()), N, max_level)
                         if nfold:
                             fold = H.empty(((nfold + 3) // 4,), dtype=torch.int32, device=dev)
                 H.check(H.lib().nr3d_lotd_bwd_dx(
-                    C.byref(m._cmeta()), N, H.F32, gcode, H.ptr(g32), gsn, gse, H.ptr(j), jsn, jse, H.ptr(dL_dx), H.ptr(gT),
-                    max_level, H.ptr(fold), st))
+                    C.byref(m._cmeta()), N, H.F32, gcode, H.ptr(g32), gsn, gse, H.ptr(j), jsn, jse, H.ptr(dL_dx),
+                    H.ptr(gT if gT_direct is None else gT_direct), 0 if gT_direct is None else 1, max_level, H.ptr(fold), st))
             if need_param_grad and N > 0 and typed:
                 ws, wsb = _dparam_workspace(m, N, dev, 1)
                 if gT is not None:
                     g32, gsn, gse, gcode = gT, 1, N, H.F32
                 H.check(H.lib().nr3d_lotd_bwd_dparam_typed(
                     C.byref(m._cmeta()), H.ptr(m._dev(dev)), N, gcode, H.ptr(g32), gsn, gse, H.ptr(_f32c(input.detach())),
-                    max_level, H.F16 if native else H.F32, 1, H.ptr(dL_dparam), H.ptr(ws), wsb, H.ptr(fold), st))
+                    max_level, H.F16 if native else H.F32, 1, H.ptr(dL_dparam), H.ptr(ws), wsb, H.ptr(fold),
+                    H.ptr(gT_direct), st))
             elif need_param_grad and N > 0:
                 x32, (p32, pcode) = _f32c(input.detach()), _ptab(params)
                 nbat = _n_batches(m, p32, batch_offsets, batched)
diff --git a/nr3d_lib_amd/csrc/host_api.hip b/nr3d_lib_amd/csrc/host_api.hip
--- a/nr3d_lib_amd/csrc/host_api.hip
+++ b/nr3d_lib_amd/csrc/host_api.hip
@@ -51,6 +51,7 @@
 	 1,  1,  1,  1,  1,  1,
 	 1,  0,  1,  1,  1,  1,
 	 1,  1,  1,
+	 1,  8,
 };
 std::atomic<int64_t> g_val[NR3D_OPT_COUNT];
 static const bool g_val_init = [] {
diff --git a/nr3d_lib_amd/csrc/lotd.hip b/nr3d_lib_amd/csrc/lotd.hip
--- a/nr3d_lib_amd/csrc/lotd.hip
+++ b/nr3d_lib_amd/csrc/lotd.hip
@@ -1031,7 +1031,7 @@
                                                                  const float *__restrict__ dydx, int64_t d_sn,
                                                                  int64_t d_se, float *__restrict__ dL_dx,
                                                                  float *__restrict__ dL_dy_T, uint32_t *__restrict__ fold,
-                                                                 uint32_t gcols, uint32_t n_zero, uint32_t slot_off) {
+                                                                 uint32_t gcols, uint32_t n_zero, uint32_t slot_off, uint64_t t_levels) {
 	constexpr int TE = 32;
 	__shared__ float tile[TE][kBlock + 1];
 	__shared__ uint32_t gred[kBlock / 64];
@@ -1073,9 +1073,17 @@
 			}
 		}
 		__syncthreads();
-		if (dL_dy_T && i < N) {
+		if (dL_dy_T && i < N && t_levels == 0ull) {
 #pragma unroll 8
 			for (uint32_t e = 0; e < te; ++e) __builtin_nontemporal_store(tile[e][threadIdx.x], &dL_dy_T[(size_t)(e0 + e) * N + i]);
+		} else if (dL_dy_T && i < N) {
+			for (uint32_t e = 0; e < te; ++e) {
+				const uint32_t q = (e0 + e) >> 1;
+				if (q < 64u && ((t_levels >> q) & 1ull)) {
+					const uint32_t row = 2u * (uint32_t)__popcll(t_levels & ((1ull << q) - 1ull)) + ((e0 + e) & 1u);
+					__builtin_nontemporal_store(tile[e][threadIdx.x], &dL_dy_T[(size_t)row * N + i]);
+				}
+			}
 		}
 		if (i < N) {
 			const float *jj = dydx + (int64_t)i * d_sn + (int64_t)e0 * d_se;
@@ -1476,7 +1484,7 @@
 
 extern "C" int nr3d_lotd_bwd_dx(const nr3d_lotd_meta_t *meta, uint32_t N, int x_dtype, int param_dtype, const void *dL_dy,
                                 int64_t g_sn, int64_t g_se, const void *dy_dx, int64_t d_sn, int64_t d_se, void *dL_dx,
-                                void *dL_dy_T, int32_t max_level, void *fold_buf, void *stream) {
+                                void *dL_dy_T, int dL_dy_T_direct, int32_t max_level, void *fold_buf, void *stream) {
 	NR3D_CHECK(meta != nullptr, "LoTD: meta is NULL");
 	NR3D_CHECK(x_dtype == NR3D_F32 && (param_dtype == NR3D_F32 || param_dtype == NR3D_F16), "LoTD::bwd_dx: f32 x, f32 / f16 dL_dy");
 	if (N == 0) return 0;
@@ -1489,16 +1497,22 @@
 	uint32_t gcols = 0, n_zero = 0, slot_off = 0;
 	uint32_t *fold = (fold_buf && pair_fold_layout(meta, N, max_level, gcols, n_zero, slot_off) != 0) ? (uint32_t *)fold_buf : nullptr;
 	NR3D_CHECK(!fold || row_major, "LoTD::bwd_dx: the hand-over buffer needs a contiguous, 16-byte aligned [N, E] dL_dy");
+	uint64_t t_levels = 0;
+	if (dL_dy_T && dL_dy_T_direct) {
+		NR3D_CHECK(!g_half && pair_rowmajor_applies(meta, N), "LoTD::bwd_dx: dL_dy_T_direct needs nr3d_lotd_pair_rowmajor_ok and f32 dL_dy");
+		t_levels = pair_direct_mask(meta, N, max_level);
+		if (t_levels == 0ull) dL_dy_T = nullptr;
+	}
 	prof::Scope ps(NR3D_PROF_LOTD_CONTRACT_DX, (hipStream_t)stream);
 	DISPATCH_D(meta->n_dims_to_encode, {
 		if (row_major && g_half)
 			hipLaunchKernelGGL((k_contract_dx_rowmajor<D, __half>), dim3(div_up(N, kBlock)), dim3(kBlock), 0, (hipStream_t)stream, N, E,
 			                   (const __half *)dL_dy, (const float *)dy_dx, d_sn, d_se, (float *)dL_dx, (float *)dL_dy_T, fold, gcols,
-			                   n_zero, slot_off);
+			                   n_zero, slot_off, t_levels);
 		else if (row_major)
 			hipLaunchKernelGGL((k_contract_dx_rowmajor<D, float>), dim3(div_up(N, kBlock)), dim3(kBlock), 0, (hipStream_t)stream, N, E,
 			                   (const float *)dL_dy, (const float *)dy_dx, d_sn, d_se, (float *)dL_dx, (float *)dL_dy_T, fold, gcols,
-			                   n_zero, slot_off);
+			                   n_zero, slot_off, t_levels);
 		else
 			hipLaunchKernelGGL(k_contract_dx<D>, dim3(div_up(N, kBlock)), dim3(kBlock), 0, (hipStream_t)stream, N, E,
 			                   (const float *)dL_dy, g_sn, g_se, (const float *)dy_dx, d_sn, d_se, (float *)dL_dx);
@@ -1561,6 +1575,9 @@
 	return fwd_lds_levels(meta, n_points, 0x7fffffff);
 }
 
+extern "C" int nr3d_lotd_pair_rowmajor_ok(const nr3d_lotd_meta_t *meta, uint32_t n_points) {
+	return pair_rowmajor_applies(meta, n_points) ? 1 : 0;
+}
 extern "C" int nr3d_lotd_pair_direct_levels(const nr3d_lotd_meta_t *meta, uint32_t n_points) {
 	return (meta && pair_applies(meta)) ? (int)pair_direct_levels(meta, n_points) : 0;
 }
@@ -1568,7 +1585,7 @@
 extern "C" int nr3d_lotd_bwd_dparam_typed(const nr3d_lotd_meta_t *meta, const void *meta_dev, uint32_t N, int grad_dtype,
                                           const void *dL_dy, int64_t g_sn, int64_t g_se, const void *x, int32_t max_level,
                                           int out_dtype, int assign, void *dL_dparam, void *workspace, uint64_t workspace_bytes,
-                                          void *fold, void *stream) {
+                                          void *fold, const void *dL_dy_T_direct, void *stream) {
 	if (int rc = check_common(meta, meta_dev, NR3D_F32, NR3D_F32)) return rc;
 	NR3D_CHECK((grad_dtype == NR3D_F32 || grad_dtype == NR3D_F16) && (out_dtype == NR3D_F32 || out_dtype == NR3D_F16),
 	           "LoTD::bwd_dparam_typed: f32 / f16 only");
@@ -1584,6 +1601,7 @@
 	p.max_level = max_level;
 	p.workspace = workspace; p.workspace_bytes = workspace_bytes; p.st = (hipStream_t)stream;
 	p.fold = (uint32_t *)fold;
+	p.gt_direct = (const float *)dL_dy_T_direct;
 	NR3D_TRY(dparam_binned(p, handled));
 	NR3D_CHECK(handled, "LoTD::bwd_dparam_typed: the pair-record path does not apply to this meta / workspace");
 	return 0;
diff --git a/nr3d_lib_amd/csrc/lotd_bin.hip b/nr3d_lib_amd/csrc/lotd_bin.hip
--- a/nr3d_lib_amd/csrc/lotd_bin.hip
+++ b/nr3d_lib_amd/csrc/lotd_bin.hip
@@ -1538,6 +1538,10 @@
 	if (pass.assign && !p.assign)
 		NR3D_HIP_CHECK(hipMemsetAsync(p.dparam, 0, (size_t)(p.n_batches ? p.n_batches : 1u) * meta->n_params * (p.out_half ? 2 : 4), p.st));
 	if (!(N <= nc && !p.second)) p.fold = nullptr;
+	const bool pair_rows = p.gt_direct && use_pair && !p.second && !p.g_half && p.min_level <= 0 && pair_rowmajor_applies(meta, N) &&
+	                       p.g_se == 1 && p.g_sn == (int64_t)E && ((uintptr_t)p.dL_dy % 16) == 0;
+	if (p.gt_direct && !pair_rows)
+		return ::nr3d::fail("LoTD::bwd: dL_dy_T_direct needs nr3d_lotd_pair_rowmajor_ok and a contiguous, 16-byte aligned f32 [N, E] dL_dy");
 
 	for (uint32_t p0 = 0; p0 < N; p0 += nc) {
 		const uint32_t n = c.n = (N - p0) < nc ? (N - p0) : nc;
@@ -1547,6 +1551,7 @@
 		                    : p.dL_dy + (int64_t)p0 * p.g_sn;
 		c.gc = c.g_rows;
 		c.sn = p.g_sn; c.se = p.g_se;
+		c.g_direct = pair_rows ? p.gt_direct : nullptr;
 		c.ba = p.batch;
 		if (c.ba.inds) c.ba.inds += p0;
 		c.ba.first_point = p0;
@@ -1559,7 +1564,7 @@
 			gt_ready = true;
 		};
 		if (use_pair) {
-			need_gt();
+			if (!pair_rows) need_gt();
 			NR3D_TRY(pair_chunk(p, c));
 			continue;
 		}
diff --git a/nr3d_lib_amd/csrc/lotd_device.h b/nr3d_lib_amd/csrc/lotd_device.h
--- a/nr3d_lib_amd/csrc/lotd_device.h
+++ b/nr3d_lib_amd/csrc/lotd_device.h
@@ -654,6 +654,7 @@
 	hipStream_t st;
 	const ForestDev *forest;
 	uint32_t *fold;
+	const float *gt_direct;
 };
 struct DparamChunk {
 	uint32_t n;
@@ -661,6 +662,7 @@
 	const float *g_rows;
 	const float *gc;
 	int64_t sn, se;
+	const float *g_direct;
 	Batch ba;
 	uint32_t *rec, *offs, *plan_buf;
 	float *partial, *gt;
@@ -683,7 +685,7 @@
 	p.min_level = 0; p.max_level = 0x7fffffff;
 	p.dparam = (float *)dparam; p.out_half = false; p.assign = false;
 	p.workspace = nullptr; p.workspace_bytes = 0; p.st = nullptr;
-	p.forest = nullptr; p.fold = nullptr;
+	p.forest = nullptr; p.fold = nullptr; p.gt_direct = nullptr;
 	return p;
 }
 
@@ -695,6 +697,8 @@
 void pair_layout(const nr3d_lotd_meta_t *m, uint32_t n_chunk, uint64_t &rec_bytes, uint64_t &offs_bytes, uint64_t &plan_bytes,
                  uint64_t &part_bytes);
 int pair_chunk(const DparamPass &p, DparamChunk &c);
+bool pair_rowmajor_applies(const nr3d_lotd_meta_t *m, uint32_t n);
+uint64_t pair_direct_mask(const nr3d_lotd_meta_t *m, uint32_t n, int32_t max_level);
 uint64_t pair_fold_layout(const nr3d_lotd_meta_t *m, uint32_t n, int32_t max_level, uint32_t &gcols, uint32_t &zero_words,
                           uint32_t &slot_off);
 
diff --git a/nr3d_lib_amd/csrc/lotd_pair.hip b/nr3d_lib_amd/csrc/lotd_pair.hip
--- a/nr3d_lib_amd/csrc/lotd_pair.hip
+++ b/nr3d_lib_amd/csrc/lotd_pair.hip
@@ -20,7 +20,9 @@
 	uint32_t bucket_base[kPMaxLv + 1];
 	uint32_t offs_base[kPMaxLv];
 	uint32_t n_blk, n_pseudo;
-	uint32_t cap;
+	uint32_t cap[kPMaxLv];
+	uint64_t rec_base[kPMaxLv + 1];
+	uint32_t align;
 	uint32_t lg;
 	uint32_t sum_log2;
 };
@@ -29,6 +31,7 @@
 struct DirectPlan {
 	uint32_t n;
 	uint32_t qmap[kDirectMaxLv], nb[kDirectMaxLv], epb[kDirectMaxLv], shift[kDirectMaxLv];
+	uint32_t gcol[kDirectMaxLv];
 	uint32_t bucket_base[kDirectMaxLv + 1];
 	uint32_t lg, sum_log2, R, pts_per_rep;
 	uint32_t merge_min;
@@ -38,6 +41,10 @@
 constexpr uint32_t kPairBp = 1024, kPairLg = 12, kPairUnroll = 4, kDirectRotate = 8, kPairUnits = 1536;
 static bool pair_quad_enabled() { return opt::on(NR3D_OPT_PAIR_QUAD); }
 static uint32_t pair_fixed() { return opt::on(NR3D_OPT_PAIR_FIXED) ? 1u : 0u; }
+static uint32_t pair_align() {
+	const int64_t a = opt::get(NR3D_OPT_PAIR_ALIGN);
+	return (a == 2 || a == 4 || a == 8) ? (uint32_t)a : 1u;
+}
 
 __device__ __forceinline__ float pair_wp2(float wp, float Cm, float Em, float &Cuse) {
 	const float floor_c = fmaxf(1e-18f * fabsf(Em), 1e-30f);
@@ -134,6 +141,7 @@
 __device__ __forceinline__ void pair_level(const PairPlan &plan, uint32_t ql, const Lvl &L, bool active, const float (&xp)[3],
                                            float g0, float g1, uint32_t smooth, u32x4 *__restrict__ stage,
                                            uint32_t *__restrict__ hist, uint32_t *__restrict__ zero_next, uint32_t *scan_lds,
+                                           uint32_t *__restrict__ pad, uint16_t *__restrict__ shift16,
                                            u32x4 *__restrict__ dst, uint32_t *__restrict__ ob, uint32_t ob_stride,
                                            const float *__restrict__ vin = nullptr, bool quad_on = false) {
 	const uint32_t nb = plan.nb[ql];
@@ -247,10 +255,12 @@
 	}
 	__syncthreads();
 
+	const uint32_t amask = plan.align - 1u;
 	{
 		const uint32_t b = threadIdx.x;
 		const uint32_t v = (b < nb) ? hist[b] : 0u;
-		uint32_t inc = v;
+		const uint32_t vp = v | (((0u - v) & amask) << 16);
+		uint32_t inc = vp;
 #pragma unroll
 		for (int off = 1; off < 64; off <<= 1) {
 			const uint32_t t = __shfl_up(inc, off, 64);
@@ -261,7 +271,11 @@
 		uint32_t wave_off = 0;
 #pragma unroll
 		for (int k = 0; k < kPBP / 64; ++k) { const uint32_t t = scan_lds[k]; if (k < (int)(threadIdx.x >> 6)) wave_off += t; }
-		if (b <= nb) hist[b] = wave_off + inc - v;
+		if (b <= nb) {
+			const uint32_t ex = wave_off + inc - vp;
+			hist[b] = ex & 0xFFFFu;
+			if (amask) pad[b] = ex >> 16;
+		}
 		__syncthreads();
 	}
 
@@ -270,6 +284,11 @@
 		for (int m = 0; m < 4; ++m) {
 			if constexpr (QUADS) { if (!emits(m)) continue; }
 			const uint32_t pos = hist[bkt[m]] + rank[m];
+			if (amask) {
+				const uint16_t sh16 = (uint16_t)pad[bkt[m]];
+				shift16[pos] = sh16;
+				if (split) shift16[pos + 1] = sh16;
+			}
 			if (QUADS && !split && m < 2 && ((qmask >> m) & 1u)) {
 				const uint32_t wzq = (uint32_t)__float2uint_rn(wp[0] * 16777215.0f), wyq = (uint32_t)__float2uint_rn(wy * 16777215.0f);
 				stage[pos] = u32x4{(hdr[m] & 8191u) | (((wyq >> 8) & 8191u) << 13) | (4u << 26) | ((wyq >> 21) << 29),
@@ -285,8 +304,12 @@
 	__syncthreads();
 
 	const uint32_t total = hist[nb];
-	for (uint32_t v = threadIdx.x; v < total; v += kPBP) __builtin_nontemporal_store(stage[v], dst + v);
-	for (uint32_t b = threadIdx.x; b <= nb; b += kPBP) ob[(size_t)b * ob_stride] = hist[b];
+	if (amask) for (uint32_t v = threadIdx.x; v < total; v += kPBP) __builtin_nontemporal_store(stage[v], dst + v + shift16[v]);
+	else       for (uint32_t v = threadIdx.x; v < total; v += kPBP) __builtin_nontemporal_store(stage[v], dst + v);
+	for (uint32_t b = threadIdx.x; b < nb; b += kPBP) {
+		const uint32_t s = hist[b];
+		ob[(size_t)b * ob_stride] = (s + (amask ? pad[b] : 0u)) | ((hist[b + 1] - s) << 16);
+	}
 	if (zero_next) __syncthreads();
 }
 
@@ -312,13 +335,20 @@
                                                    const float *__restrict__ g, int64_t g_sn, int64_t g_se,
                                                    u32x4 *__restrict__ rec, uint32_t *__restrict__ offs_g,
                                                    uint32_t *__restrict__ gmax, DirectPlan dp, const float *__restrict__ vin_,
-                                                   uint32_t quad_on) {
+                                                   uint32_t quad_on, uint32_t mode) {
 	constexpr uint32_t kPCap = (uint32_t)kPBP * 4u;
 	extern __shared__ __attribute__((aligned(16))) uint32_t smem[];
 	__shared__ uint32_t scan_lds[kPBP / 64];
 	u32x4 *stage = reinterpret_cast<u32x4 *>(smem);
-	uint32_t *hist = smem + (size_t)kPCap * 4;
-	const uint32_t blk = blockIdx.x, ql = blockIdx.y;
+	uint16_t *shift16 = reinterpret_cast<uint16_t *>(smem + (size_t)kPCap * 4);
+	uint32_t *hist = smem + (size_t)kPCap * 4 + (plan.align > 1u ? kPCap / 2u : 0u);
+	uint32_t blk = blockIdx.x, ql = blockIdx.y;
+	if (mode & 2u) {
+		const uint32_t id = blockIdx.y * gridDim.x + blockIdx.x, per = 8u * plan.n_pseudo, grp = id / per, rem = id - grp * per;
+		const uint32_t in_grp = min(8u, plan.n_blk - grp * 8u);
+		ql = rem / in_grp;
+		blk = grp * 8u + (rem - ql * in_grp);
+	}
 	const uint32_t q = plan.qmap[ql], nb = plan.nb[ql];
 	const uint32_t level = meta_level_of(md, q);
 	const Lvl L = load_level(md, level);
@@ -330,15 +360,20 @@
 	if (active) {
 #pragma unroll
 		for (int d = 0; d < 3; ++d) xp[d] = x[(size_t)i * 3 + d];
-		g0 = g[(int64_t)i * g_sn + (int64_t)(q * 2) * g_se];
-		g1 = g[(int64_t)i * g_sn + (int64_t)(q * 2 + 1) * g_se];
+		if (mode & 1u) {
+			const float2 t = *reinterpret_cast<const float2 *>(g + (int64_t)i * g_sn + (int64_t)(q * 2));
+			g0 = t.x; g1 = t.y;
+		} else {
+			g0 = g[(int64_t)i * g_sn + (int64_t)(q * 2) * g_se];
+			g1 = g[(int64_t)i * g_sn + (int64_t)(q * 2 + 1) * g_se];
+		}
 		if constexpr (SECOND) {
 #pragma unroll
 			for (int d = 0; d < 3; ++d) vin[d] = vin_[(size_t)i * 3 + d];
 		}
 	}
-	pair_level<kPBP, SECOND>(plan, ql, L, active, xp, g0, g1, smooth, stage, hist, nullptr, scan_lds,
-	                         rec + ((size_t)ql * plan.n_blk + blk) * (size_t)plan.cap, offs_g + plan.offs_base[ql] + blk, plan.n_blk, vin,
+	pair_level<kPBP, SECOND>(plan, ql, L, active, xp, g0, g1, smooth, stage, hist, nullptr, scan_lds, hist + (nb + 1u), shift16,
+	                         rec + plan.rec_base[ql] + (size_t)blk * plan.cap[ql], offs_g + plan.offs_base[ql] + blk, plan.n_blk, vin,
 	                         quad_on != 0u);
 	if (gmax) {
 		uint32_t gbits;
@@ -406,9 +441,8 @@
 			uint32_t q = 0;
 			while (q + 1 < plan.n_pseudo && plan.bucket_base[q + 1] <= fb) ++q;
 			const uint32_t *ob0 = offs_g + plan.offs_base[q] + (size_t)(fb - plan.bucket_base[q]) * plan.n_blk;
-			const uint32_t *ob1 = ob0 + plan.n_blk;
 			uint32_t sum = 0;
-			for (uint32_t blk = lane; blk < plan.n_blk; blk += 64) sum += ob1[blk] - ob0[blk];
+			for (uint32_t blk = lane; blk < plan.n_blk; blk += 64) sum += ob0[blk] >> 16;
 #pragma unroll
 			for (int off = 32; off >= 1; off >>= 1) sum += __shfl_xor(sum, off, 64);
 			if (lane == 0) __hip_atomic_store(tot + fb, sum, __ATOMIC_RELAXED, __HIP_MEMORY_SCOPE_AGENT);
@@ -581,16 +615,15 @@
 	constexpr uint32_t n_waves = kPAccThreads / 64;
 	const uint32_t blk_lo = 0u, blk_hi = (plan.n_blk > r) ? (plan.n_blk - r + R - 1u) / R : 0u;
 	const uint32_t *ob0 = offs_g + plan.offs_base[q] + (size_t)b * plan.n_blk;
-	const uint32_t *ob1 = ob0 + plan.n_blk;
-	const uint32_t kPCap = plan.cap;
-	const u32x4 *rec_q = rec + (size_t)q * plan.n_blk * (size_t)kPCap;
+	const uint32_t kPCap = plan.cap[q];
+	const u32x4 *rec_q = rec + plan.rec_base[q];
 	const uint32_t per_wave = (blk_hi - blk_lo + n_waves - 1) / n_waves;
 	const uint32_t w_lo = min(blk_lo + wave * per_wave, blk_hi), w_hi = min(w_lo + per_wave, blk_hi);
 	constexpr int kGroup = 8;
 	for (uint32_t blk0 = w_lo; blk0 < w_hi; blk0 += 64) {
 		const uint32_t mb = blk0 + lane;
-		const uint32_t s_l = (mb < w_hi) ? ob0[r + R * mb] : 0u;
-		const uint32_t e_l = (mb < w_hi) ? ob1[r + R * mb] : 0u;
+		const uint32_t o_l = (mb < w_hi) ? ob0[r + R * mb] : 0u;
+		const uint32_t s_l = o_l & 0xFFFFu, e_l = s_l + (o_l >> 16);
 		const uint32_t n_run = min(64u, w_hi - blk0);
 		const u32x4 *rec_b = rec_q + (size_t)(r + R * blk0) * kPCap;
 		for (uint32_t j0 = 0; j0 < n_run; j0 += kGroup) {
@@ -737,7 +770,7 @@
 			float xp[3];
 #pragma unroll
 			for (int d = 0; d < 3; ++d) xp[d] = x[(size_t)i * 3 + d];
-			const float g0 = g[(int64_t)i * g_sn + (int64_t)(q * 2) * g_se], g1 = g[(int64_t)i * g_sn + (int64_t)(q * 2 + 1) * g_se];
+			const float g0 = g[(int64_t)i * g_sn + (int64_t)dp.gcol[e] * g_se], g1 = g[(int64_t)i * g_sn + (int64_t)(dp.gcol[e] + 1u) * g_se];
 			uint32_t hdr[4], bkt[4], cell[3];
 			constexpr int kW = SECOND ? 3 : 0;
 			float A[4][2], wp[SECOND ? 4 : 1], vin[3] = {0.0f, 0.0f, 0.0f};
@@ -934,9 +967,9 @@
 
 
 static void pair_plan(const nr3d_lotd_meta_t *m, uint32_t n_chunk, int32_t min_level, int32_t max_level, PairPlan &plan,
-                      uint64_t &offs_words, uint64_t skip_pseudo = 0) {
+                      uint64_t &offs_words, uint64_t skip_pseudo = 0, uint32_t align = pair_align()) {
 	plan.n_blk = div_up(n_chunk, kPairBp);
-	plan.cap = kPairBp * 4u;
+	plan.align = align;
 	plan.lg = kPairLg;
 	plan.sum_log2 = 3;
 	while ((1ull << (plan.sum_log2 - 3)) < n_chunk) ++plan.sum_log2;
@@ -961,8 +994,11 @@
 		plan.bucket_base[nq] = nq ? plan.bucket_base[nq - 1] + plan.nb[nq - 1] : 0u;
 		plan.offs_base[nq] = (uint32_t)base;
 		base += (uint64_t)(nb + 1) * plan.n_blk;
+		plan.cap[nq] = (kPairBp * 4u + (plan.align - 1u) * nb + 7u) & ~7u;
+		plan.rec_base[nq] = nq ? plan.rec_base[nq - 1] + (uint64_t)plan.n_blk * plan.cap[nq - 1] : 0ull;
 		++nq;
 	}
+	plan.rec_base[nq] = nq ? plan.rec_base[nq - 1] + (uint64_t)plan.n_blk * plan.cap[nq - 1] : 0ull;
 	plan.n_pseudo = nq;
 	plan.bucket_base[nq] = nq ? plan.bucket_base[nq - 1] + plan.nb[nq - 1] : 0u;
 	offs_words = base;
@@ -980,6 +1016,7 @@
 		if (dp.bucket_base[dp.n] + full.nb[ql] > kDirectMaxWg) break;
 		const uint32_t e = dp.n++;
 		dp.qmap[e] = full.qmap[ql]; dp.nb[e] = full.nb[ql]; dp.epb[e] = full.epb[ql]; dp.shift[e] = full.shift[ql];
+		dp.gcol[e] = 2u * full.qmap[ql];
 		dp.bucket_base[e + 1] = dp.bucket_base[e] + full.nb[ql];
 		mask |= 1ull << full.qmap[ql];
 	}
@@ -994,6 +1031,18 @@
 	return mask;
 }
 
+bool pair_rowmajor_applies(const nr3d_lotd_meta_t *m, uint32_t n) {
+	return opt::get(NR3D_OPT_PAIR_ROWMAJOR) == 1 && m && pair_applies(m) && n != 0 && dparam_one_pass(n) &&
+	       2u * m->n_pseudo_levels == m->n_encoded_dims;
+}
+uint64_t pair_direct_mask(const nr3d_lotd_meta_t *m, uint32_t n, int32_t max_level) {
+	PairPlan plan;
+	uint64_t ow;
+	pair_plan(m, n, 0, max_level, plan, ow);
+	DirectPlan dp;
+	return plan.n_pseudo ? pair_direct_plan(plan, n, dp) : 0ull;
+}
+
 uint32_t pair_direct_levels(const nr3d_lotd_meta_t *m, uint32_t n_points) {
 	PairPlan plan;
 	uint64_t ow;
@@ -1007,9 +1056,9 @@
                  uint64_t &part_bytes) {
 	PairPlan plan;
 	uint64_t ow;
-	pair_plan(m, n_chunk, 0, 0x7fffffff, plan, ow);
+	pair_plan(m, n_chunk, 0, 0x7fffffff, plan, ow, 0, 8u);
 	const uint32_t NB = plan.bucket_base[plan.n_pseudo];
-	rec_bytes = (uint64_t)plan.n_pseudo * plan.n_blk * plan.cap * 16;
+	rec_bytes = plan.rec_base[plan.n_pseudo] * 16;
 	offs_bytes = ((ow * 4 + 255) / 256) * 256;
 	plan_bytes = (((uint64_t)NB * 3 + 4) * 4 + 255) / 256 * 256;
 	part_bytes = (uint64_t)(kPairUnits + NB + kDirectMaxWg) * (2u << plan.lg) * 4;
@@ -1045,6 +1094,8 @@
 	const int32_t min_level = p.min_level, max_level = p.max_level;
 	const float *x = c.xc, *g = c.gc, *vin = p.second ? c.vc : nullptr;
 	const int64_t g_sn = c.sn, g_se = c.se;
+	const bool rows = c.g_direct != nullptr;
+	const uint32_t bin_mode = (rows ? 1u : 0u) | ((rows || opt::get(NR3D_OPT_PAIR_ROWMAJOR) == 2) ? 2u : 0u);
 	uint32_t *offs = c.offs, *plan_buf = c.plan_buf, *fold = p.fold;
 	float *dparam = p.dparam, *partial = c.partial;
 	hipStream_t st = p.st;
@@ -1062,6 +1113,8 @@
 	{
 		const uint64_t skip = pair_direct_plan(pl, n, dp);
 		if (skip) pair_plan(meta, n, min_level, max_level, pl, ow, skip);
+		if (rows)
+			for (uint32_t e = 0; e < dp.n; ++e) dp.gcol[e] = 2u * e;
 	}
 	uint32_t nb_max = 0;
 	for (uint32_t q = 0; q < pl.n_pseudo; ++q) nb_max = nb_max > pl.nb[q] ? nb_max : pl.nb[q];
@@ -1069,17 +1122,17 @@
 	uint32_t *tot = plan_buf, *rep = plan_buf + NB, *item_start = plan_buf + 2 * (size_t)NB;
 	uint32_t *gmax = fold ? fold : plan_buf + 3 * (size_t)NB + 2;
 	uint32_t *bticket = fold ? fold + kFoldHead : nullptr;
-	const size_t bin_lds_max = (size_t)kPairBp * 4 * 16 + (size_t)(kPMaxNb + 2) * 8;
+	const size_t bin_lds_max = (size_t)kPairBp * 4 * (16 + 2) + (size_t)(kPMaxNb + 2) * 8;
 	static LdsOnce once_bin, once_acc;
 	NR3D_TRY(NR3D_LDS_LIMIT(once_bin, c.dev, (int)bin_lds_max, k_pair_bin<kPairBp>, k_pair_bin<kPairBp, true>));
 	NR3D_TRY(NR3D_LDS_LIMIT(once_acc, c.dev, kPLdsMax * 8, k_pair_direct<true>, k_pair_direct<false>, k_pair_direct<true, true>,
 	                        k_pair_direct<false, true>, k_pair_accum<kPairUnroll, false>, k_pair_accum<kPairUnroll, true>));
 	if (!fold) NR3D_HIP_CHECK(hipMemsetAsync(gmax, 0, 2 * sizeof(uint32_t), st));
-	const size_t bin_lds = (size_t)kPairBp * 4 * 16 + (size_t)(nb_max + 1) * 4;
+	const size_t bin_lds = (size_t)kPairBp * 4 * (pl.align > 1u ? 18 : 16) + (size_t)(nb_max + 1) * (pl.align > 1u ? 8 : 4);
 	const uint32_t quad_on = (!vin && pair_quad_enabled()) ? 1u : 0u;
 #define NR3D_PAIR_BIN(BP) if (vin) NR3D_PAIR_BIN_(BP, true); else NR3D_PAIR_BIN_(BP, false)
 #define NR3D_PAIR_BIN_(BP, SEC) hipLaunchKernelGGL((k_pair_bin<BP, SEC>), dim3(pl.n_blk, pl.n_pseudo), dim3(BP), bin_lds, st, pl, md, n, max_level, \
-	meta->interpolation_type, x, g, g_sn, g_se, (u32x4 *)c.rec, offs, fold ? nullptr : gmax, dp, vin, quad_on)
+	meta->interpolation_type, x, g, g_sn, g_se, (u32x4 *)c.rec, offs, fold ? nullptr : gmax, dp, vin, quad_on, bin_mode)
 	{
 		prof::Scope ps(NR3D_PROF_LOTD_BIN, st);
 		NR3D_PAIR_BIN(kPairBp);
@@ -1095,7 +1148,8 @@
 		prof::Scope ps(NR3D_PROF_LOTD_DIRECT, st);
 		auto direct = [&](auto kern) {
 			hipLaunchKernelGGL(kern, dim3(dp.R, nbk_direct + plan_rows), dim3(kPAccThreads), (size_t)(16u << pl.lg), st, dp, md, n, max_level,
-			                   meta->interpolation_type, x, g, g_sn, g_se, gmax, dpart, vin, plan_rows, pl, offs, units, tot, rep, item_start,
+			                   meta->interpolation_type, x, rows ? c.g_direct : g, rows ? (int64_t)1 : g_sn, rows ? (int64_t)n : g_se, gmax, dpart, vin,
+			                   plan_rows, pl, offs, units, tot, rep, item_start,
 			                   gmax + 1, slots, n_slots, fold, empty_one);
 		};
 		if (vin) { if (pair_fixed()) direct(k_pair_direct<true, true>); else direct(k_pair_direct<false, true>); }
```

New measurement: 1131 Mpoints/s. 0.983x the previous value.
